# yichuan-w/LEANN

Hardware: AMD Instinct MI355X
Metric: queries/sec at recall@10>=0.9, 1M-chunk HNSW, MiniLM-L6 recompute (higher is better)
Workload: dtype fp16

## Files before the change

### include/leann_mi355x.h

```cpp
#ifndef LEANN_MI355X_H
#define LEANN_MI355X_H

#include <stddef.h>
#include <stdint.h>

#ifdef __cplusplus
extern "C" {
#endif

#define LM_OK 0
#define LM_EINVAL (-1)
#define LM_ENOENT (-2)
#define LM_EFORMAT (-3)
#define LM_EHIP (-4)
#define LM_ESTATE (-5)
#define LM_EPROVIDER (-6)

#define LM_METRIC_INNER_PRODUCT 0
#define LM_METRIC_L2 1

#define LM_DTYPE_F32 0
#define LM_DTYPE_F16 1

typedef struct lm_index lm_index;
typedef struct lm_tokens lm_tokens;

const char *lm_last_error(void);
int lm_device_count(void);
const char *lm_version(void);
#define LM_ABI_REVISION 6
int lm_abi_revision(void);

int lm_index_read(const char *path, int device, lm_index **out);

int lm_index_create_from_csr(int64_t ntotal, int32_t d, int32_t metric,
                             const uint64_t *node_offsets ,
                             const uint64_t *level_ptr, int64_t n_level_ptr,
                             const int32_t *neighbors, int64_t n_neighbors,
                             const int32_t *levels ,
                             int32_t entry_point, int32_t max_level, int device, lm_index **out);

typedef struct {
    const int32_t *d_nodes;
    const int32_t *d_adj;
    int64_t n_rows;
    int32_t cap;
} lm_graph_level;
int lm_index_create_view(int64_t ntotal, int32_t d, int32_t metric, const lm_graph_level *levels ,
                         int32_t n_levels, int32_t entry_point, int device, lm_index **out);
void lm_index_free(lm_index *idx);

typedef struct {
    int64_t ntotal;
    int32_t d;
    int32_t d_padded;
    int32_t metric;
    int32_t entry_point;
    int32_t max_level;
    int32_t max_degree0;
    int32_t max_degree_up;
    int64_t n_neighbors;
    int32_t has_table;
    int32_t has_provider;
    int32_t device;
} lm_index_info_t;
int lm_index_info(const lm_index *idx, lm_index_info_t *out);

int lm_index_attach_table(lm_index *idx, const void *table, int32_t dtype, int64_t ntotal, int32_t d,
                          int32_t location);

typedef int (*lm_provider_fn)(void *user, const int32_t *d_ids, int32_t n, void **d_out, void *stream);
int lm_index_set_provider(lm_index *idx, lm_provider_fn fn, void *user);

int lm_index_set_hub_cache(lm_index *idx, const int32_t *ids, int32_t n, const float *d_embeddings);

int lm_index_set_stream(lm_index *idx, void *hip_stream);

typedef struct {
    int32_t efSearch;
    int32_t beam_size;
    int32_t check_relative_distance;
    float pq_pruning_ratio;
    int32_t local_prune;
    float send_neigh_times_ratio;
    int32_t batch_size;
    int32_t zmq_port;
    int32_t recompute;
    int32_t max_batch;
    int32_t recompute_memo;
} lm_search_params;
void lm_search_params_default(lm_search_params *p);

int lm_index_search(lm_index *idx, int64_t n, const float *x, int32_t k, float *distances,
                    int64_t *labels, const lm_search_params *params);
int lm_index_search_device(lm_index *idx, int64_t n, const float *d_x, int32_t k, float *d_distances,
                           int64_t *d_labels, const lm_search_params *params);

typedef struct {
    int64_t ndis;
    int64_t nunique;
    int64_t nrounds;
    int64_t nexpand;
    int64_t update_launches;
    double update_ms;
    double expand_ms;
    double provider_ms;
    int64_t nadc;
    double update_span_ms;
    int64_t update_span_launches;
} lm_search_stats;
int lm_index_get_stats(const lm_index *idx, lm_search_stats *out);
int lm_index_set_profiling(lm_index *idx, int32_t enable);
int lm_index_event_overhead_us(lm_index *idx, double *out_us);
int lm_index_set_option(lm_index *idx, const char *name, int64_t value);
int lm_index_get_option(const lm_index *idx, const char *name, int64_t *value);

int lm_pq_attach(lm_index *idx, int32_t m, const float *codebooks, const uint8_t *codes, int64_t ntotal);
int lm_pq_attach_chunked(lm_index *idx, int32_t m, const int32_t *chunk_offsets, const float *codebooks, const uint8_t *codes,
                         int64_t ntotal);
typedef struct {
    int32_t complexity;
    int32_t beam_width;
    int32_t num_threads;
    int32_t use_deferred_fetch;
    int32_t skip_search_reorder;
    int32_t recompute_neighbors;
    int32_t dedup_node_dis;
    float prune_ratio;
    int32_t batch_recompute;
    int32_t use_global_pruning;
} lm_pq_search_params;
void lm_pq_search_params_default(lm_pq_search_params *p);
int lm_pq_batch_search(lm_index *idx, int64_t n, const float *x, int32_t k, const lm_pq_search_params *params,
                       int64_t *labels, float *distances);
int lm_pq_batch_search_device(lm_index *idx, int64_t n, const float *d_x, int32_t k,
                              const lm_pq_search_params *params, int64_t *d_labels, float *d_distances);

int lm_dist_gather(const void *d_table, int32_t dtype, int32_t d_padded, int32_t metric,
                   const float *d_q, const int32_t *d_qidx, const int32_t *d_ids, int64_t npairs,
                   float *d_out, void *stream);
int lm_topk_merge(const int64_t *d_in_ids, const float *d_in_dist, int32_t S, int32_t B, int32_t k,
                  int32_t metric, int64_t *d_out_ids, float *d_out_dist, void *stream);
#define LM_SELECT_MAX_K 512
int lm_select_neighbors(const void *d_table, int32_t dtype, int64_t ntable, int32_t d_padded, int32_t metric,
                        const int32_t *d_cand, const float *d_dist, int64_t n, int32_t K, int32_t m, float alpha,
                        uint8_t *d_keep, void *stream);
#define LM_LINK_STAGE 128
size_t lm_graph_add_links_workspace_bytes(int64_t n, int64_t ne);
int lm_graph_add_links(const void *d_table, int32_t dtype, int32_t d_padded, int32_t metric, int32_t *d_adj, float *d_dist,
                       int32_t *d_deg, int64_t n, int32_t cap, const int32_t *d_src, const int32_t *d_dst, const float *d_w, int64_t ne,
                       float alpha, void *d_workspace, size_t workspace_bytes, void *stream);
size_t lm_graph_prune_hubs_workspace_bytes(int64_t n, int32_t cap, int32_t m_low, int64_t n_hubs);
int lm_graph_prune_hubs(const void *d_table, int32_t dtype, int32_t d_padded, int32_t metric, const int32_t *d_adj_in, int64_t n,
                        int32_t cap, int32_t m_low, int64_t n_hubs, float alpha, int32_t *d_adj_out, float *d_dist_out,
                        int32_t *d_deg_out, int32_t *d_hubs , int32_t *d_indeg ,
                        void *d_workspace, size_t workspace_bytes, void *stream);
int lm_graph_insert_batch(lm_index *view, const int32_t *d_batch, int64_t b, int32_t replace, int32_t kk, int32_t m, float alpha,
                          const lm_search_params *params, int32_t *d_adj, float *d_dist, int32_t *d_deg,
                          int32_t *d_cand_out , float *d_cdist_out , uint8_t *d_keep_out );
#define LM_EXACT_MAX_K 256
size_t lm_exact_search_workspace_bytes(int64_t ntable, int64_t nq, int32_t k);
int lm_exact_search(const void *d_table, int32_t dtype, int64_t ntable, int32_t d_padded, int32_t metric, const float *d_q, int64_t nq,
                    int32_t k, const uint32_t *d_allow, float *d_distances, int64_t *d_labels, void *d_workspace, size_t workspace_bytes,
                    void *stream);
int lm_index_search_exact(lm_index *idx, int64_t n, const float *x, int32_t k, const uint32_t *allow, float *distances, int64_t *labels);
int lm_index_search_exact_device(lm_index *idx, int64_t n, const float *d_x, int32_t k, const uint32_t *d_allow, float *d_distances,
                                 int64_t *d_labels);
int lm_index_search_filtered(lm_index *idx, int64_t n, const float *x, int32_t k, const uint32_t *allow, float *distances, int64_t *labels,
                             const lm_search_params *params);
int lm_index_search_filtered_device(lm_index *idx, int64_t n, const float *d_x, int32_t k, const uint32_t *d_allow, float *d_distances,
                                    int64_t *d_labels, const lm_search_params *params);
#define LM_PQ_FLAT_MAX_L 1024
size_t lm_pq_scan_workspace_bytes(int64_t ntotal, int64_t nq, int32_t m, int32_t L);
int lm_pq_scan(const uint8_t *d_codes, int64_t ntotal, int32_t m, const int32_t *chunk_offsets, const float *d_codebooks, int32_t d,
               int32_t metric, const float *d_q, int64_t nq, int32_t ldq, int32_t L, const uint32_t *d_allow, float *d_distances,
               int64_t *d_labels, void *d_workspace, size_t workspace_bytes, void *stream);
int lm_pq_flat_search(lm_index *idx, int64_t n, const float *x, int32_t k, const lm_pq_search_params *params, const uint32_t *allow,
                      int64_t *labels, float *distances);
int lm_pq_flat_search_device(lm_index *idx, int64_t n, const float *d_x, int32_t k, const lm_pq_search_params *params,
                             const uint32_t *d_allow, int64_t *d_labels, float *d_distances);
int lm_pq_batch_search_filtered(lm_index *idx, int64_t n, const float *x, int32_t k, const lm_pq_search_params *params,
                                const uint32_t *allow, int64_t *labels, float *distances);
int lm_pq_batch_search_filtered_device(lm_index *idx, int64_t n, const float *d_x, int32_t k, const lm_pq_search_params *params,
                                       const uint32_t *d_allow, int64_t *d_labels, float *d_distances);
#define LM_PQ_MAX_SUB 64
int lm_pq_encode(const void *d_x, int32_t dtype, int64_t n, int32_t ld, int32_t d, int32_t m, const int32_t *chunk_offsets,
                 const float *d_codebooks, uint8_t *d_codes, void *stream);
int lm_pq_train(const void *d_x, int32_t dtype, int64_t s, int32_t ld, int32_t d, int32_t m, const int32_t *chunk_offsets,
                int32_t iters, float *d_codebooks, void *d_workspace, size_t workspace_bytes, void *stream);
size_t lm_pq_train_workspace_bytes(int64_t s, int32_t d, int32_t m);

int lm_add_layernorm_f16(const void *d_x, const void *d_residual, const void *d_gamma, const void *d_beta,
                         void *d_out, int64_t rows, int32_t hidden, float eps, void *stream);

int lm_attn_varlen_hd32_f16(const void *d_qkv, const int32_t *d_cu_seqlens, int32_t n_seqs, int32_t heads,
                            int32_t max_len, void *d_out, void *stream);

int lm_attn_varlen_f16(const void *d_qkv, const int32_t *d_cu_seqlens, int32_t n_seqs, int32_t heads, int32_t head_dim,
                       int32_t max_len, void *d_out, void *stream);

int lm_embed_layernorm_f16(const int32_t *d_tok, const int32_t *d_pos, const void *d_word, const void *d_pos_table,
                           const void *d_type0, const void *d_gamma, const void *d_beta, void *d_out, int64_t rows,
                           int32_t hidden, float eps, void *stream);

int lm_pack_tokens(const int32_t *d_ids, const int32_t *d_lens, const int32_t *d_cu_seqlens, int32_t n, int32_t t,
                   int32_t *d_tok, int32_t *d_pos, void *stream);

int lm_meanpool_varlen_f16(const void *d_x, const int32_t *d_cu_seqlens, int32_t n_seqs, int32_t hidden,
                           int32_t normalize, float *d_out, void *stream);

int lm_layer_tail_h384_f16(const void *d_attn, const void *d_resid, const void *d_wo_img, const float *d_bo,
                           const void *d_gamma1, const void *d_beta1, float eps1, const void *d_w1_img, const float *d_b1,
                           const void *d_w2_img, const float *d_b2, const void *d_gamma, const void *d_beta, void *d_out,
                           int64_t tokens, int32_t ffn, float eps, void *stream);
int lm_layer_tail_pack_h384(const void *d_wo_slabs, const void *d_w1_acc, const void *d_w2_slabs, int32_t ffn, void *d_wo_img,
                            void *d_w1_img, void *d_w2_img, void *stream);

int lm_qkv_attn_h384_f16(const void *d_x, const void *d_wqkv_img, const float *d_bqkv, const int32_t *d_cu_seqlens, int32_t n_seqs, int32_t max_len,
                         int64_t total_tokens, void *d_out, void *stream);
int lm_h384_first_half_form(int32_t heads, int32_t max_len, int64_t total_tokens, int32_t n_seqs);

int lm_qkv_h384_f16(const void *d_x, const void *d_w_img, const float *d_bias, int32_t n_out, void *d_out, int64_t tokens,
                    void *stream);
int lm_qkv_pack_h384(const void *d_w, int32_t n_out, void *d_w_img, void *stream);

int lm_gemm_ws_h384_f16(const void *d_x, const void *d_w, const float *d_bias, int32_t n_out, void *d_out, int64_t tokens,
                        void *stream);

int lm_gemm_f16(const void *d_x, const void *d_w, const float *d_bias, const void *d_residual, int32_t epilogue, int32_t n_out,
                int32_t k_in, void *d_out, int64_t tokens, void *stream);

typedef struct lm_bert_h384_layer {
    const void *wqkv;
    const float *bqkv;
    const void *wo_img;
    const float *bo;
    const void *ln1_gamma, *ln1_beta;
    const void *w1_img;
    const float *b1;
    const void *w2_img;
    const float *b2;
    const void *ln2_gamma, *ln2_beta;
    const void *wo, *w1, *w2;
    const void *wqkv_img;
} lm_bert_h384_layer;
#define LM_BERT_SMALL_TOKENS 8192
#define LM_BERT_QKV_GEMM_TOKENS 45056

typedef struct lm_bert_h384 {
    int32_t n_layers, heads, ffn, normalize;
    int32_t pooling;
    float ln_eps;
    const void *word, *pos_table, *type0, *emb_gamma, *emb_beta;
    const lm_bert_h384_layer *layers;
} lm_bert_h384;

size_t lm_bert_h384_workspace_bytes(int64_t total_tokens);
int lm_bert_h384_forward_packed(const lm_bert_h384 *m, const int32_t *d_tok, const int32_t *d_pos, const int32_t *d_cu_seqlens,
                                int32_t n_seqs, int64_t total_tokens, int32_t max_len, void *d_workspace, size_t workspace_bytes,
                                float *d_out, void *stream);

typedef struct lm_bert_layer {
    const void *wqkv;
    const float *bqkv;
    const void *wo;
    const float *bo;
    const void *ln1_gamma, *ln1_beta;
    const void *w1;
    const float *b1;
    const void *w2;
    const float *b2;
    const void *ln2_gamma, *ln2_beta;
} lm_bert_layer;

typedef struct lm_bert {
    int32_t hidden, n_layers, heads, ffn;
    int32_t pooling;
    int32_t normalize;
    float ln_eps;
    const void *word, *pos_table, *type0, *emb_gamma, *emb_beta;
    const lm_bert_layer *layers;
} lm_bert;

size_t lm_bert_workspace_bytes(const lm_bert *m, int64_t total_tokens);
int lm_bert_forward_packed(const lm_bert *m, const int32_t *d_tok, const int32_t *d_pos, const int32_t *d_cu_seqlens, int32_t n_seqs,
                           int64_t total_tokens, int32_t max_len, void *d_workspace, size_t workspace_bytes, float *d_out, void *stream);
int lm_clspool_varlen_f16(const void *d_x, const int32_t *d_cu_seqlens, int32_t n_seqs, int32_t hidden, int32_t normalize,
                          float *d_out, void *stream);

int lm_tokens_create(const uint16_t *tokens, const uint64_t *offsets , int64_t n, int device,
                     lm_tokens **out);
void lm_tokens_free(lm_tokens *t);
int lm_tokens_gather(const lm_tokens *t, const int32_t *d_ids, int32_t n, int32_t T, int32_t pad_id,
                     int32_t *d_out_ids, int32_t *d_out_len, void *stream);
int64_t lm_tokens_count(const lm_tokens *t);

typedef struct lm_recompute lm_recompute;
typedef struct lm_recompute_stats {
    int64_t calls, chunks, tokens, forwards, host_syncs;
} lm_recompute_stats;
int lm_recompute_create(const lm_bert_h384 *model, const lm_tokens *tokens, int32_t max_seq_len, int64_t max_tokens_per_forward,
                        lm_recompute **out);
int lm_recompute_create_general(const lm_bert *model, const lm_tokens *tokens, int32_t max_seq_len, int64_t max_tokens_per_forward,
                                lm_recompute **out);
void lm_recompute_free(lm_recompute *rc);
int lm_recompute_provider(void *user, const int32_t *d_ids, int32_t n, void **d_out, void *stream);
int lm_recompute_embed(lm_recompute *rc, const int32_t *d_ids, int32_t n, float *d_out, void *stream);
int lm_recompute_get_stats(const lm_recompute *rc, lm_recompute_stats *out);
int lm_index_set_recompute(lm_index *idx, lm_recompute *rc);

#define LM_KT_LAYER_TAIL 0
#define LM_KT_GEMM_WS 1
#define LM_KT_ATTN 2
#define LM_KT_GEMM_F16 3
#define LM_KT_QKV 4
#define LM_KT_QKV_ATTN 5
#define LM_KT_COUNT 6
typedef struct lm_kernel_time {
    const char *name;
    int64_t launches;
    double ms, work;
} lm_kernel_time;
int lm_kernel_timing_enable(uint32_t mask);
int lm_kernel_timing_read(lm_kernel_time *out, int32_t capacity, int32_t reset);

#ifdef __cplusplus
}
#endif
#endif
```

### leann_amd/_lib.py

```python

from __future__ import annotations

import ctypes as C
from pathlib import Path

_PKG = Path(__file__).resolve().parent
LIB_PATH = _PKG / "lib" / "libleann_mi355x.so"
BUILD_LIB_PATH = _PKG / "lib" / "libleann_hnswbuild.so"

LM_OK, LM_EINVAL, LM_ENOENT, LM_EFORMAT, LM_EHIP, LM_ESTATE, LM_EPROVIDER = 0, -1, -2, -3, -4, -5, -6
METRIC_INNER_PRODUCT, METRIC_L2 = 0, 1
DTYPE_F32, DTYPE_F16 = 0, 1
SELECT_MAX_K = 512
PQ_MAX_SUB = 64
EXACT_MAX_K = 256
LINK_STAGE = 128
PQ_FLAT_MAX_L = 1024


class LeannMi355xError(RuntimeError):
    pass


class IndexInfo(C.Structure):
    _fields_ = [
        ("ntotal", C.c_int64), ("d", C.c_int32), ("d_padded", C.c_int32), ("metric", C.c_int32),
        ("entry_point", C.c_int32), ("max_level", C.c_int32), ("max_degree0", C.c_int32),
        ("max_degree_up", C.c_int32), ("n_neighbors", C.c_int64), ("has_table", C.c_int32),
        ("has_provider", C.c_int32), ("device", C.c_int32),
    ]


class GraphLevel(C.Structure):
    _fields_ = [("d_nodes", C.c_void_p), ("d_adj", C.c_void_p), ("n_rows", C.c_int64), ("cap", C.c_int32)]


class SearchParams(C.Structure):

    _fields_ = [
        ("efSearch", C.c_int32), ("beam_size", C.c_int32), ("check_relative_distance", C.c_int32),
        ("pq_pruning_ratio", C.c_float), ("local_prune", C.c_int32), ("send_neigh_times_ratio", C.c_float),
        ("batch_size", C.c_int32), ("zmq_port", C.c_int32), ("recompute", C.c_int32), ("max_batch", C.c_int32),
        ("recompute_memo", C.c_int32),
    ]


class SearchStats(C.Structure):
    _fields_ = [
        ("ndis", C.c_int64), ("nunique", C.c_int64), ("nrounds", C.c_int64), ("nexpand", C.c_int64),
        ("update_launches", C.c_int64), ("update_ms", C.c_double), ("expand_ms", C.c_double),
        ("provider_ms", C.c_double), ("nadc", C.c_int64), ("update_span_ms", C.c_double), ("update_span_launches", C.c_int64),
    ]


class PqSearchParams(C.Structure):

    _fields_ = [
        ("complexity", C.c_int32), ("beam_width", C.c_int32), ("num_threads", C.c_int32),
        ("use_deferred_fetch", C.c_int32), ("skip_search_reorder", C.c_int32), ("recompute_neighbors", C.c_int32),
        ("dedup_node_dis", C.c_int32), ("prune_ratio", C.c_float), ("batch_recompute", C.c_int32),
        ("use_global_pruning", C.c_int32),
    ]


class BertH384Layer(C.Structure):
    _fields_ = [(n, C.c_void_p) for n in ("wqkv", "bqkv", "wo_img", "bo", "ln1_gamma", "ln1_beta", "w1_img", "b1", "w2_img", "b2", "ln2_gamma", "ln2_beta",
                                          "wo", "w1", "w2", "wqkv_img")]


class BertH384(C.Structure):
    _fields_ = [("n_layers", C.c_int32), ("heads", C.c_int32), ("ffn", C.c_int32), ("normalize", C.c_int32), ("pooling", C.c_int32), ("ln_eps", C.c_float),
                ("word", C.c_void_p), ("pos_table", C.c_void_p), ("type0", C.c_void_p), ("emb_gamma", C.c_void_p), ("emb_beta", C.c_void_p),
                ("layers", C.POINTER(BertH384Layer))]


class BertLayer(C.Structure):
    _fields_ = [(n, C.c_void_p) for n in ("wqkv", "bqkv", "wo", "bo", "ln1_gamma", "ln1_beta", "w1", "b1", "w2", "b2", "ln2_gamma", "ln2_beta")]


class Bert(C.Structure):
    _fields_ = [("hidden", C.c_int32), ("n_layers", C.c_int32), ("heads", C.c_int32), ("ffn", C.c_int32), ("pooling", C.c_int32),
                ("normalize", C.c_int32), ("ln_eps", C.c_float),
                ("word", C.c_void_p), ("pos_table", C.c_void_p), ("type0", C.c_void_p), ("emb_gamma", C.c_void_p), ("emb_beta", C.c_void_p),
                ("layers", C.POINTER(BertLayer))]


class KernelTime(C.Structure):
    _fields_ = [("name", C.c_char_p), ("launches", C.c_int64), ("ms", C.c_double), ("work", C.c_double)]


KT_LAYER_TAIL, KT_GEMM_WS, KT_ATTN, KT_GEMM_F16, KT_QKV, KT_QKV_ATTN, KT_COUNT = 0, 1, 2, 3, 4, 5, 6


class RecomputeStats(C.Structure):
    _fields_ = [(n, C.c_int64) for n in ("calls", "chunks", "tokens", "forwards", "host_syncs")]


ABI_REVISION = 6

PROVIDER_FN = C.CFUNCTYPE(C.c_int, C.c_void_p, C.c_void_p, C.c_int32, C.POINTER(C.c_void_p), C.c_void_p)

EXPORTED_SYMBOLS = [
    "lm_last_error", "lm_device_count", "lm_version", "lm_abi_revision",
    "lm_index_read", "lm_index_create_from_csr", "lm_index_create_view", "lm_index_free", "lm_index_info",
    "lm_index_attach_table", "lm_index_set_provider", "lm_index_set_hub_cache", "lm_index_set_stream",
    "lm_search_params_default", "lm_index_search", "lm_index_search_device",
    "lm_index_get_stats", "lm_index_set_profiling", "lm_index_set_option", "lm_index_get_option", "lm_index_event_overhead_us",
    "lm_dist_gather", "lm_topk_merge", "lm_select_neighbors", "lm_graph_add_links", "lm_graph_add_links_workspace_bytes", "lm_graph_prune_hubs", "lm_graph_prune_hubs_workspace_bytes", "lm_graph_insert_batch", "lm_pq_encode", "lm_pq_train", "lm_pq_train_workspace_bytes",
    "lm_exact_search", "lm_exact_search_workspace_bytes", "lm_index_search_exact", "lm_index_search_exact_device",
    "lm_index_search_filtered", "lm_index_search_filtered_device",
    "lm_pq_scan", "lm_pq_scan_workspace_bytes", "lm_pq_flat_search", "lm_pq_flat_search_device",
    "lm_pq_attach", "lm_pq_attach_chunked", "lm_pq_search_params_default", "lm_pq_batch_search", "lm_pq_batch_search_device",
    "lm_pq_batch_search_filtered", "lm_pq_batch_search_filtered_device",
    "lm_add_layernorm_f16", "lm_attn_varlen_hd32_f16", "lm_attn_varlen_f16", "lm_embed_layernorm_f16", "lm_meanpool_varlen_f16",
    "lm_layer_tail_h384_f16", "lm_layer_tail_pack_h384", "lm_qkv_h384_f16", "lm_qkv_attn_h384_f16", "lm_h384_first_half_form", "lm_qkv_pack_h384", "lm_gemm_ws_h384_f16", "lm_gemm_f16", "lm_pack_tokens",
    "lm_tokens_create", "lm_tokens_free", "lm_tokens_gather", "lm_tokens_count",
    "lm_bert_h384_workspace_bytes", "lm_bert_h384_forward_packed",
    "lm_bert_workspace_bytes", "lm_bert_forward_packed", "lm_clspool_varlen_f16",
    "lm_recompute_create", "lm_recompute_create_general", "lm_recompute_free", "lm_recompute_provider", "lm_recompute_embed", "lm_recompute_get_stats", "lm_index_set_recompute",
    "lm_kernel_timing_enable", "lm_kernel_timing_read",
]

_lib = None


def load() -> C.CDLL:
    global _lib
    if _lib is not None:
        return _lib
    if not LIB_PATH.exists():
        raise LeannMi355xError(
            f"{LIB_PATH} is missing: build it with `python -c 'import __graft_entry__ as g; g.build()'` "
            "or `make -C leann_amd/csrc`. leann-backend-mi355x has no CPU fallback."
        )
    lib = C.CDLL(str(LIB_PATH))
    vp, i32, i64, f32p = C.c_void_p, C.c_int32, C.c_int64, C.c_void_p
    lib.lm_last_error.restype = C.c_char_p
    lib.lm_version.restype = C.c_char_p
    if lib.lm_abi_revision() != ABI_REVISION:
        raise LeannMi355xError(f"{LIB_PATH} speaks ABI revision {lib.lm_abi_revision()}, this package was written against {ABI_REVISION}: rebuild it "
                               "(`make -C leann_amd/csrc`)")
    lib.lm_device_count.restype = C.c_int
    lib.lm_index_read.argtypes = [C.c_char_p, C.c_int, C.POINTER(vp)]
    lib.lm_index_create_from_csr.argtypes = [i64, i32, i32, vp, vp, i64, vp, i64, vp, i32, i32, C.c_int, C.POINTER(vp)]
    lib.lm_index_create_view.argtypes = [i64, i32, i32, C.POINTER(GraphLevel), i32, i32, C.c_int, C.POINTER(vp)]
    lib.lm_index_free.argtypes = [vp]
    lib.lm_index_free.restype = None
    lib.lm_index_info.argtypes = [vp, C.POINTER(IndexInfo)]
    lib.lm_index_attach_table.argtypes = [vp, vp, i32, i64, i32, i32]
    lib.lm_index_set_provider.argtypes = [vp, PROVIDER_FN, vp]
    lib.lm_index_set_stream.argtypes = [vp, vp]
    lib.lm_index_set_hub_cache.argtypes = [vp, vp, i32, vp]
    lib.lm_search_params_default.argtypes = [C.POINTER(SearchParams)]
    lib.lm_search_params_default.restype = None
    lib.lm_index_search.argtypes = [vp, i64, f32p, i32, vp, vp, C.POINTER(SearchParams)]
    lib.lm_index_search_device.argtypes = [vp, i64, vp, i32, vp, vp, C.POINTER(SearchParams)]
    lib.lm_index_get_stats.argtypes = [vp, C.POINTER(SearchStats)]
    lib.lm_index_set_profiling.argtypes = [vp, i32]
    lib.lm_index_set_option.argtypes = [vp, C.c_char_p, i64]
    lib.lm_index_get_option.argtypes = [vp, C.c_char_p, C.POINTER(C.c_int64)]
    lib.lm_index_event_overhead_us.argtypes = [vp, C.POINTER(C.c_double)]
    lib.lm_dist_gather.argtypes = [vp, i32, i32, i32, vp, vp, vp, i64, vp, vp]
    lib.lm_topk_merge.argtypes = [vp, vp, i32, i32, i32, i32, vp, vp, vp]
    lib.lm_select_neighbors.argtypes = [vp, i32, i64, i32, i32, vp, vp, i64, i32, i32, C.c_float, vp, vp]
    lib.lm_graph_add_links_workspace_bytes.argtypes = [i64, i64]
    lib.lm_graph_add_links_workspace_bytes.restype = C.c_size_t
    lib.lm_graph_add_links.argtypes = [vp, i32, i32, i32, vp, vp, vp, i64, i32, vp, vp, vp, i64, C.c_float, vp, C.c_size_t, vp]
    lib.lm_graph_prune_hubs_workspace_bytes.argtypes = [i64, i32, i32, i64]
    lib.lm_graph_prune_hubs_workspace_bytes.restype = C.c_size_t
    lib.lm_graph_prune_hubs.argtypes = [vp, i32, i32, i32, vp, i64, i32, i32, i64, C.c_float, vp, vp, vp, vp, vp, vp, C.c_size_t, vp]
    lib.lm_graph_insert_batch.argtypes = [vp, vp, i64, i32, i32, i32, C.c_float, C.POINTER(SearchParams), vp, vp, vp, vp, vp, vp]
    lib.lm_pq_encode.argtypes = [vp, i32, i64, i32, i32, i32, vp, vp, vp, vp]
    lib.lm_pq_train.argtypes = [vp, i32, i64, i32, i32, i32, vp, i32, vp, vp, C.c_size_t, vp]
    lib.lm_pq_train_workspace_bytes.argtypes = [i64, i32, i32]
    lib.lm_pq_train_workspace_bytes.restype = C.c_size_t
    lib.lm_exact_search_workspace_bytes.argtypes = [i64, i64, i32]
    lib.lm_exact_search_workspace_bytes.restype = C.c_size_t
    lib.lm_exact_search.argtypes = [vp, i32, i64, i32, i32, vp, i64, i32, vp, vp, vp, vp, C.c_size_t, vp]
    lib.lm_index_search_exact.argtypes = [vp, i64, vp, i32, vp, vp, vp]
    lib.lm_index_search_exact_device.argtypes = [vp, i64, vp, i32, vp, vp, vp]
    lib.lm_index_search_filtered.argtypes = [vp, i64, vp, i32, vp, vp, vp, C.POINTER(SearchParams)]
    lib.lm_index_search_filtered_device.argtypes = [vp, i64, vp, i32, vp, vp, vp, C.POINTER(SearchParams)]
    lib.lm_pq_scan_workspace_bytes.argtypes = [i64, i64, i32, i32]
    lib.lm_pq_scan_workspace_bytes.restype = C.c_size_t
    lib.lm_pq_scan.argtypes = [vp, i64, i32, vp, vp, i32, i32, vp, i64, i32, i32, vp, vp, vp, vp, C.c_size_t, vp]
    lib.lm_pq_flat_search.argtypes = [vp, i64, vp, i32, C.POINTER(PqSearchParams), vp, vp, vp]
    lib.lm_pq_flat_search_device.argtypes = [vp, i64, vp, i32, C.POINTER(PqSearchParams), vp, vp, vp]
    lib.lm_pq_attach.argtypes = [vp, i32, vp, vp, i64]
    lib.lm_pq_attach_chunked.argtypes = [vp, i32, vp, vp, vp, i64]
    lib.lm_pq_search_params_default.argtypes = [C.POINTER(PqSearchParams)]
    lib.lm_pq_search_params_default.restype = None
    lib.lm_pq_batch_search.argtypes = [vp, i64, vp, i32, C.POINTER(PqSearchParams), vp, vp]
    lib.lm_pq_batch_search_device.argtypes = [vp, i64, vp, i32, C.POINTER(PqSearchParams), vp, vp]
    lib.lm_pq_batch_search_filtered.argtypes = [vp, i64, vp, i32, C.POINTER(PqSearchParams), vp, vp, vp]
    lib.lm_pq_batch_search_filtered_device.argtypes = [vp, i64, vp, i32, C.POINTER(PqSearchParams), vp, vp, vp]
    lib.lm_add_layernorm_f16.argtypes = [vp, vp, vp, vp, vp, i64, i32, C.c_float, vp]
    lib.lm_attn_varlen_hd32_f16.argtypes = [vp, vp, i32, i32, i32, vp, vp]
    lib.lm_attn_varlen_f16.argtypes = [vp, vp, i32, i32, i32, i32, vp, vp]
    lib.lm_embed_layernorm_f16.argtypes = [vp, vp, vp, vp, vp, vp, vp, vp, i64, i32, C.c_float, vp]
    lib.lm_meanpool_varlen_f16.argtypes = [vp, vp, i32, i32, i32, vp, vp]
    lib.lm_layer_tail_h384_f16.argtypes = [vp, vp, vp, vp, vp, vp, C.c_float, vp, vp, vp, vp, vp, vp, vp, i64, i32, C.c_float, vp]
    lib.lm_layer_tail_pack_h384.argtypes = [vp, vp, vp, i32, vp, vp, vp, vp]
    lib.lm_qkv_h384_f16.argtypes = [vp, vp, vp, i32, vp, i64, vp]
    lib.lm_qkv_attn_h384_f16.argtypes = [vp, vp, vp, vp, i32, i32, i64, vp, vp]
    lib.lm_h384_first_half_form.argtypes = [i32, i32, i64, i32]
    lib.lm_qkv_pack_h384.argtypes = [vp, i32, vp, vp]
    lib.lm_gemm_ws_h384_f16.argtypes = [vp, vp, vp, i32, vp, i64, vp]
    lib.lm_gemm_f16.argtypes = [vp, vp, vp, vp, i32, i32, i32, vp, i64, vp]
    lib.lm_pack_tokens.argtypes = [vp, vp, vp, i32, i32, vp, vp, vp]
    lib.lm_tokens_create.argtypes = [vp, vp, i64, C.c_int, C.POINTER(vp)]
    lib.lm_tokens_free.argtypes = [vp]
    lib.lm_tokens_free.restype = None
    lib.lm_tokens_gather.argtypes = [vp, vp, i32, i32, i32, vp, vp, vp]
    lib.lm_tokens_count.argtypes = [vp]
    lib.lm_tokens_count.restype = i64
    lib.lm_bert_h384_workspace_bytes.argtypes = [i64]
    lib.lm_bert_h384_workspace_bytes.restype = C.c_size_t
    lib.lm_bert_h384_forward_packed.argtypes = [C.POINTER(BertH384), vp, vp, vp, i32, i64, i32, vp, C.c_size_t, vp, vp]
    lib.lm_bert_workspace_bytes.argtypes = [C.POINTER(Bert), i64]
    lib.lm_bert_workspace_bytes.restype = C.c_size_t
    lib.lm_bert_forward_packed.argtypes = [C.POINTER(Bert), vp, vp, vp, i32, i64, i32, vp, C.c_size_t, vp, vp]
    lib.lm_clspool_varlen_f16.argtypes = [vp, vp, i32, i32, i32, vp, vp]
    lib.lm_recompute_create.argtypes = [C.POINTER(BertH384), vp, i32, i64, C.POINTER(vp)]
    lib.lm_recompute_create_general.argtypes = [C.POINTER(Bert), vp, i32, i64, C.POINTER(vp)]
    lib.lm_recompute_free.argtypes = [vp]
    lib.lm_recompute_free.restype = None
    lib.lm_recompute_provider.argtypes = [vp, vp, i32, C.POINTER(vp), vp]
    lib.lm_recompute_embed.argtypes = [vp, vp, i32, vp, vp]
    lib.lm_recompute_get_stats.argtypes = [vp, C.POINTER(RecomputeStats)]
    lib.lm_index_set_recompute.argtypes = [vp, vp]
    lib.lm_kernel_timing_enable.argtypes = [C.c_uint32]
    lib.lm_kernel_timing_read.argtypes = [C.POINTER(KernelTime), i32, i32]
    _lib = lib
    return lib


def last_error() -> str:
    return (load().lm_last_error() or b"").decode("utf-8", "replace")


def check(rc: int, what: str = "") -> None:
    if rc == LM_OK:
        return
    msg = f"{what}: {last_error()}" if what else last_error()
    if rc == LM_EINVAL or rc == LM_EFORMAT:
        raise ValueError(msg)
    if rc == LM_ENOENT:
        raise FileNotFoundError(msg)
    raise LeannMi355xError(msg)


def kernel_timing_enable(mask: int) -> None:
    check(load().lm_kernel_timing_enable(int(mask)), "lm_kernel_timing_enable")


def kernel_timing_read(reset: bool = False) -> dict:
    arr = (KernelTime * KT_COUNT)()
    check(load().lm_kernel_timing_read(arr, KT_COUNT, 1 if reset else 0), "lm_kernel_timing_read")
    return {a.name.decode(): {"launches": int(a.launches), "ms": float(a.ms), "work": float(a.work)} for a in arr}


def device_count() -> int:
    return int(load().lm_device_count())


def require_gpu() -> None:
    if device_count() <= 0:
        raise LeannMi355xError("no HIP device visible: leann-backend-mi355x needs an MI355X (gfx950) GPU and has no CPU fallback")
```

### leann_amd/csrc/lm_device_types.h

```cpp
#pragma once

namespace lm {

struct L0Range {
    uint64_t begin;
    uint32_t count;
    uint32_t pad;
};

struct GraphDev {
    int64_t N;
    int32_t entry_point, max_level;
    const uint64_t* node_offsets;
    const uint64_t* level_ptr;
    const int32_t* neighbors;
    const L0Range* l0;
};

struct WsDev {
    int32_t B, ef, W, maxnew;
    int32_t efs;
    int32_t batch;
    int32_t check_rel;
    int64_t nw;
    int32_t* phase;
    int32_t* level;
    uint64_t* cur_key;
    int32_t* nsteps;
    int32_t* npool;
    int32_t* npop;
    int32_t* nnew;
    unsigned long long* ndis_q;
    int32_t* pop;
    int32_t* newid;
    uint64_t* pool;
    uint32_t* visited;
    uint32_t* rbm;
    uint32_t* rbm_snap;
    int32_t* word_rank;
    int32_t* tile_sum;
    int32_t* uniq;
    uint64_t* aq;
    int32_t* naq;
    unsigned long long* nadc_q;
    int32_t* memo_slot;
    float* memo;
    unsigned long long* counters;
};
enum { C_LIVE = 0, C_NUNIQ = 1, C_NDIS = 2, C_NEXPAND = 3, C_ROUNDS = 4, C_RC_TOKENS = 5, C_NADC = 6, C_RC_MAXLEN = 7, C_PQ_OVERFLOW = 8, C_PQ_ALLOWED = 9, C_NCOUNTERS = 10 };

constexpr int UNIQ_TILE = 4096;
constexpr int AQ_CAP = 512;


}
```

### leann_amd/csrc/lm_encoder_forward.cpp

```cpp
#include <algorithm>
#include <cstdint>
#include <cstdlib>
#include <string>

#include "lm_internal.h"

static int64_t small_tokens_limit() {
    const char* e = getenv("LEANN_MI355X_SMALL_TOKENS");
    return e ? (int64_t)atoll(e) : (int64_t)LM_BERT_SMALL_TOKENS;
}

lm::H384FirstHalf lm::h384_first_half_form(int32_t heads, int32_t max_len, int64_t total_tokens, int32_t n_seqs) {
    auto is = [](const char* name, char c) {
        const char* e = getenv(name);
        return e && e[0] == c;
    };
    if (heads != 12 || max_len > 256) return H384_PAIR_ROW_MAJOR;
    if (is("LEANN_MI355X_QKV_LAYOUT", '0') || is("LEANN_MI355X_ATTN3", '9') || is("LEANN_MI355X_ATTN", '2')) return H384_PAIR_ROW_MAJOR;
    if (is("LEANN_MI355X_FUSED_QKV_ATTN", '0')) return H384_PAIR_HEAD_MAJOR;
    if (is("LEANN_MI355X_FUSED_QKV_ATTN", '1')) return H384_FUSED;
    return n_seqs > 0 && total_tokens >= (int64_t)H384_FUSED_MIN_MEAN_LEN * n_seqs ? H384_FUSED : H384_PAIR_HEAD_MAJOR;
}
extern "C" int lm_h384_first_half_form(int32_t heads, int32_t max_len, int64_t total_tokens, int32_t n_seqs) {
    return (int)lm::h384_first_half_form(heads, max_len, total_tokens, n_seqs);
}

static int64_t qkv_gemm_tokens_limit() {
    if (const char* e = getenv("LEANN_MI355X_QKV_GEMM_TOKENS")) return (int64_t)atoll(e);
    const char* s = getenv("LEANN_MI355X_SMALL_TOKENS");
    return s && atoll(s) == 0 ? 0 : (int64_t)LM_BERT_QKV_GEMM_TOKENS;
}

extern "C" size_t lm_bert_h384_workspace_bytes(int64_t total_tokens) {
    if (total_tokens <= 0) return 0;
    const size_t small = total_tokens <= std::max<int64_t>(small_tokens_limit(), LM_BERT_SMALL_TOKENS) ? (size_t)total_tokens * 2560 * 2 : 0;
    return (size_t)total_tokens * (3 * 384 + 1152) * 2 + small;
}

extern "C" int lm_bert_h384_forward_packed(const lm_bert_h384* m, const int32_t* d_tok, const int32_t* d_pos, const int32_t* d_cu_seqlens,
                                           int32_t n_seqs, int64_t total_tokens, int32_t max_len, void* d_workspace, size_t workspace_bytes,
                                           float* d_out, void* stream) {
    using namespace lm;
    if (n_seqs == 0 || total_tokens == 0) return LM_OK;
    if (!m || !m->layers || !d_tok || !d_pos || !d_cu_seqlens || !d_workspace || !d_out || n_seqs < 0 || total_tokens < 0)
        LM_FAIL(LM_EINVAL, "lm_bert_h384_forward_packed: bad arguments");
    if (!bert_h384_envelope_ok(m->n_layers, m->heads, m->ffn)) LM_FAIL(LM_EINVAL, "lm_bert_h384_forward_packed: needs " LM_BERT_H384_ENVELOPE_TEXT);
    if (max_len <= 0 || max_len > 256) LM_FAIL(LM_EINVAL, "lm_bert_h384_forward_packed: sequence lengths 1..256");
    if (m->pooling != 0 && m->pooling != 1) LM_FAIL(LM_EINVAL, "lm_bert_h384_forward_packed: pooling 0 (mean) or 1 (CLS)");
    if (workspace_bytes < lm_bert_h384_workspace_bytes(total_tokens)) LM_FAIL(LM_EINVAL, "lm_bert_h384_forward_packed: workspace too small");
    const size_t row = (size_t)total_tokens * 384 * 2;
    unsigned char* ws = (unsigned char*)d_workspace;
    void* x = ws;
    void* a = ws + row;
    void* y = ws + 2 * row;
    void* qkv = ws + 3 * row;
    int rc = lm_embed_layernorm_f16(d_tok, d_pos, m->word, m->pos_table, m->type0, m->emb_gamma, m->emb_beta, x, total_tokens, 384, m->ln_eps, stream);
    if (rc) return rc;
    bool small = total_tokens <= small_tokens_limit() && m->ffn % 128 == 0;
    for (int l = 0; small && l < m->n_layers; ++l) small = m->layers[l].wo && m->layers[l].w1 && m->layers[l].w2;
    void* hid = ws + 3 * row + (size_t)total_tokens * 1152 * 2;
    H384FirstHalf first_half = h384_first_half_form(m->heads, max_len, total_tokens, n_seqs);
    bool qkv_gemm = !small && total_tokens <= qkv_gemm_tokens_limit();
    for (int l = 0; qkv_gemm && l < m->n_layers; ++l) qkv_gemm = m->layers[l].wqkv != nullptr;
    {
        const char* f = getenv("LEANN_MI355X_FUSED_QKV_ATTN");
        if (qkv_gemm && f && f[0] == '1') qkv_gemm = false;
        else if (qkv_gemm) first_half = H384_PAIR_ROW_MAJOR;
    }
    for (int l = 0; l < m->n_layers; ++l) {
        const lm_bert_h384_layer& L = m->layers[l];
        if (small) {
            if ((rc = lm_gemm_f16(x, L.wqkv, L.bqkv, nullptr, 0, 1152, 384, qkv, total_tokens, stream))) return rc;
            if ((rc = lm_attn_varlen_hd32_f16(qkv, d_cu_seqlens, n_seqs, m->heads, max_len, a, stream))) return rc;
            if ((rc = lm_gemm_f16(a, L.wo, L.bo, x, 2, 384, 384, y, total_tokens, stream))) return rc;
            if ((rc = lm_add_layernorm_f16(y, nullptr, L.ln1_gamma, L.ln1_beta, x, total_tokens, 384, m->ln_eps, stream))) return rc;
            if ((rc = lm_gemm_f16(x, L.w1, L.b1, nullptr, 1, m->ffn, 384, hid, total_tokens, stream))) return rc;
            if ((rc = lm_gemm_f16(hid, L.w2, L.b2, x, 2, 384, m->ffn, y, total_tokens, stream))) return rc;
            if ((rc = lm_add_layernorm_f16(y, nullptr, L.ln2_gamma, L.ln2_beta, x, total_tokens, 384, m->ln_eps, stream))) return rc;
            continue;
        }
        if (L.wqkv_img && first_half == H384_FUSED) {
            if ((rc = lm_qkv_attn_h384_launch(x, L.wqkv_img, L.bqkv, d_cu_seqlens, n_seqs, max_len, total_tokens, a, stream))) return rc;
        } else if (L.wqkv_img && first_half == H384_PAIR_HEAD_MAJOR) {
            if ((rc = lm_qkv_h384_launch(x, L.wqkv_img, L.bqkv, 1152, qkv, total_tokens, 1, stream))) return rc;
            if ((rc = lm_attn_v3_launch_hd32(qkv, d_cu_seqlens, n_seqs, m->heads, max_len, a, total_tokens, stream))) return rc;
        } else {
            if ((rc = qkv_gemm      ? lm_gemm_f16(x, L.wqkv, L.bqkv, nullptr, 0, 1152, 384, qkv, total_tokens, stream)
                      : L.wqkv_img ? lm_qkv_h384_f16(x, L.wqkv_img, L.bqkv, 1152, qkv, total_tokens, stream)
                                   : lm_gemm_ws_h384_f16(x, L.wqkv, L.bqkv, 1152, qkv, total_tokens, stream)))
                return rc;
            if ((rc = lm_attn_varlen_hd32_f16(qkv, d_cu_seqlens, n_seqs, m->heads, max_len, a, stream))) return rc;
        }
        if ((rc = lm_layer_tail_h384_f16(a, x, L.wo_img, L.bo, L.ln1_gamma, L.ln1_beta, m->ln_eps, L.w1_img, L.b1, L.w2_img, L.b2, L.ln2_gamma,
                                         L.ln2_beta, y, total_tokens, m->ffn, m->ln_eps, stream)))
            return rc;
        void* t = x;
        x = y;
        y = t;
    }
    return m->pooling == 1 ? lm_clspool_varlen_f16(x, d_cu_seqlens, n_seqs, 384, m->normalize, d_out, stream)
                           : lm_meanpool_varlen_f16(x, d_cu_seqlens, n_seqs, 384, m->normalize, d_out, stream);
}

static const char* bert_envelope(const lm_bert* m) {
    if (!m || !m->layers || m->n_layers <= 0) return "NULL model / no layers";
    if (m->hidden <= 0 || m->hidden % 128 || m->hidden > 768) return "hidden must be a multiple of 128, <= 768";
    if (m->ffn <= 0 || m->ffn % 128) return "ffn must be a multiple of 128";
    if (m->heads <= 0 || (m->heads * 32 != m->hidden && m->heads * 64 != m->hidden)) return "head_dim = hidden / heads must be 32 or 64";
    if (m->pooling != 0 && m->pooling != 1) return "pooling: 0 = mean, 1 = CLS";
    return nullptr;
}

extern "C" size_t lm_bert_workspace_bytes(const lm_bert* m, int64_t total_tokens) {
    if (!m || total_tokens <= 0) return 0;
    return (size_t)total_tokens * ((size_t)6 * m->hidden + m->ffn) * 2;
}

extern "C" int lm_bert_forward_packed(const lm_bert* m, const int32_t* d_tok, const int32_t* d_pos, const int32_t* d_cu_seqlens, int32_t n_seqs,
                                      int64_t total_tokens, int32_t max_len, void* d_workspace, size_t workspace_bytes, float* d_out,
                                      void* stream) {
    using namespace lm;
    if (n_seqs == 0 || total_tokens == 0) return LM_OK;
    if (const char* why = bert_envelope(m)) LM_FAIL(LM_EINVAL, std::string("lm_bert_forward_packed: ") + why);
    if (!d_tok || !d_pos || !d_cu_seqlens || !d_workspace || !d_out || n_seqs < 0 || total_tokens < 0)
        LM_FAIL(LM_EINVAL, "lm_bert_forward_packed: bad arguments");
    const int32_t H = m->hidden, hd = H / m->heads;
    if (max_len <= 0 || max_len > (hd == 32 ? 256 : 512)) LM_FAIL(LM_EINVAL, "lm_bert_forward_packed: sequence lengths 1..256 (head_dim 32) / 1..512 (head_dim 64)");
    if (workspace_bytes < lm_bert_workspace_bytes(m, total_tokens)) LM_FAIL(LM_EINVAL, "lm_bert_forward_packed: workspace too small");
    const size_t row = (size_t)total_tokens * H * 2;
    unsigned char* ws = (unsigned char*)d_workspace;
    void *x = ws, *a = ws + row, *y = ws + 2 * row, *qkv = ws + 3 * row, *hid = ws + 6 * row;
    int rc = lm_embed_layernorm_f16(d_tok, d_pos, m->word, m->pos_table, m->type0, m->emb_gamma, m->emb_beta, x, total_tokens, H, m->ln_eps, stream);
    if (rc) return rc;
    for (int l = 0; l < m->n_layers; ++l) {
        const lm_bert_layer& L = m->layers[l];
        if ((rc = lm_gemm_f16(x, L.wqkv, L.bqkv, nullptr, 0, 3 * H, H, qkv, total_tokens, stream))) return rc;
        if ((rc = hd == 32 ? lm_attn_varlen_hd32_f16(qkv, d_cu_seqlens, n_seqs, m->heads, max_len, a, stream)
                           : lm_attn_varlen_f16(qkv, d_cu_seqlens, n_seqs, m->heads, hd, max_len, a, stream)))
            return rc;
        if ((rc = lm_gemm_f16(a, L.wo, L.bo, x, 2, H, H, y, total_tokens, stream))) return rc;
        if ((rc = lm_add_layernorm_f16(y, nullptr, L.ln1_gamma, L.ln1_beta, x, total_tokens, H, m->ln_eps, stream))) return rc;
        if ((rc = lm_gemm_f16(x, L.w1, L.b1, nullptr, 1, m->ffn, H, hid, total_tokens, stream))) return rc;
        if ((rc = lm_gemm_f16(hid, L.w2, L.b2, x, 2, H, m->ffn, y, total_tokens, stream))) return rc;
        if ((rc = lm_add_layernorm_f16(y, nullptr, L.ln2_gamma, L.ln2_beta, x, total_tokens, H, m->ln_eps, stream))) return rc;
    }
    return m->pooling == 1 ? lm_clspool_varlen_f16(x, d_cu_seqlens, n_seqs, H, m->normalize, d_out, stream)
                           : lm_meanpool_varlen_f16(x, d_cu_seqlens, n_seqs, H, m->normalize, d_out, stream);
}
```

### leann_amd/csrc/lm_internal.h

```cpp
#pragma once
#include <hip/hip_runtime.h>

#include <cstdint>
#include <cstdio>
#include <string>
#include <vector>

#include "../../include/leann_mi355x.h"

namespace lm {

void set_error(const std::string& msg);

#define LM_HIP(expr)                                                                       \
    do {                                                                                   \
        hipError_t _e = (expr);                                                            \
        if (_e != hipSuccess) {                                                            \
            lm::set_error(std::string(#expr) + ": " + hipGetErrorString(_e));              \
            return LM_EHIP;                                                                \
        }                                                                                  \
    } while (0)

#ifndef LM_KEEP_LOCAL
#define LM_KEEP_LOCAL(v) asm volatile("" : "+v"(v))
#endif

#ifndef LM_ONE_WAVE_PER_SIMD
#define LM_ONE_WAVE_PER_SIMD __attribute__((amdgpu_waves_per_eu(1, 1)))
#endif
#ifndef LM_TWO_WAVES_PER_SIMD
#define LM_TWO_WAVES_PER_SIMD __attribute__((amdgpu_waves_per_eu(2, 2)))
#endif

#ifndef LM_WAVE_SYNC
#define LM_WAVE_SYNC() ((void)0)
#endif

#define LM_FAIL(code, msg)        \
    do {                          \
        lm::set_error(msg);       \
        return (code);            \
    } while (0)

struct DynLdsAttr {
    size_t bytes[32] = {};
};
inline hipError_t ensure_dyn_lds(DynLdsAttr& a, const void* fn, size_t bytes) {
    int dev = 0;
    if (hipGetDevice(&dev) != hipSuccess || dev < 0) dev = 0;
    size_t& have = a.bytes[dev & 31];
    if (bytes <= have && dev < 32) return hipSuccess;
    hipError_t e = hipFuncSetAttribute(fn, hipFuncAttributeMaxDynamicSharedMemorySize, (int)bytes);
    if (e == hipSuccess) have = bytes;
    return e;
}

struct KtScope {
    int kid;
    void* st;
    double work;
    void* a;
    int dev;
    KtScope(int kid, void* stream, double work);
    ~KtScope();
    KtScope(const KtScope&) = delete;
    KtScope& operator=(const KtScope&) = delete;
};

void kt_attn_work(const int32_t* d_cu_seqlens, int32_t n_seqs, int32_t hidden, void* stream, int kid = LM_KT_ATTN);

enum : int32_t { PH_SEED = 0, PH_UPPER = 1, PH_BEAM = 2, PH_DONE = 3 };

constexpr uint64_t KEY_NONE = 0xFFFFFFFFFFFFFFFFull;
constexpr uint64_t KEY_EXPANDED = 1ull;

__host__ __device__ inline uint64_t make_key(float d, int32_t id) {
    if (d != d) d = __builtin_inff();
    if (d == 0.0f) d = 0.0f;
    uint32_t u = __builtin_bit_cast(uint32_t, d);
    u ^= (u >> 31) ? 0xFFFFFFFFu : 0x80000000u;
    return ((uint64_t)u << 32) | ((uint64_t)(uint32_t)id << 1);
}
__host__ __device__ inline float key_dist(uint64_t key) {
    uint32_t u = (uint32_t)(key >> 32);
    u ^= (u >> 31) ? 0x80000000u : 0xFFFFFFFFu;
    return __builtin_bit_cast(float, u);
}
__host__ __device__ inline int32_t key_id(uint64_t key) { return (int32_t)((uint32_t)key >> 1); }

struct HostCsr {
    int64_t ntotal = 0;
    int32_t d = 0;
    int32_t metric = 0;
    int32_t entry_point = -1;
    int32_t max_level = -1;
    std::vector<int32_t> levels;
    std::vector<uint64_t> level_ptr;
    std::vector<uint64_t> node_offsets;
    std::vector<int32_t> neighbors;
    std::vector<float> storage;
};
int read_csr_file(const char* path, HostCsr& out);

}

struct lm_tokens {
    int device = 0;
    int64_t n = 0;
    uint64_t total = 0;
    uint16_t* d_tok = nullptr;
    uint64_t* d_off = nullptr;
};

struct lm_recompute;
namespace lm {
int rc_prepare(lm_recompute* rc, const int32_t* d_ids, const unsigned long long* d_n, int64_t cap, unsigned long long* d_total,
               unsigned long long* d_maxlen, hipStream_t st);
void rc_prepared(lm_recompute* rc, const int32_t* d_ids, int32_t n, int64_t total, int32_t max_len);
int32_t rc_width(const lm_recompute* rc);
inline bool bert_h384_envelope_ok(int n_layers, int heads, int ffn) { return n_layers > 0 && heads * 32 == 384 && ffn >= 192 && ffn <= 1728 && ffn % 192 == 0; }
#define LM_BERT_H384_ENVELOPE_TEXT "hidden 384 = heads x 32 and ffn a multiple of 192 in [192, 1728]"
enum H384FirstHalf : int { H384_FUSED = 0, H384_PAIR_HEAD_MAJOR = 1, H384_PAIR_ROW_MAJOR = 2 };
constexpr int H384_FUSED_MIN_MEAN_LEN = 216;
H384FirstHalf h384_first_half_form(int32_t heads, int32_t max_len, int64_t total_tokens, int32_t n_seqs);

}

int lm_qkv_h384_launch(const void* d_x, const void* d_w_img, const float* d_bias, int32_t n_out, void* d_out, int64_t tokens, int32_t head_major, void* stream);

int lm_attn_v3_launch_hd32(const void* d_qkv, const int32_t* d_cu_seqlens, int32_t n_seqs, int32_t heads, int32_t max_len, void* d_out, int64_t total_tokens,
                           void* stream);

int lm_qkv_attn_h384_launch(const void* d_x, const void* d_wqkv_img, const float* d_bqkv, const int32_t* d_cu_seqlens, int32_t n_seqs, int32_t max_len,
                            int64_t total_tokens, void* d_out, void* stream);

int lm_add_layernorm_r16_launch(const void* d_x, const void* d_residual, const void* d_gamma, const void* d_beta, void* d_out,
                                int64_t rows, int32_t hidden, float eps, void* stream);
```

### leann_amd/csrc/lm_recompute.hip

```cpp
#include <algorithm>
#include <climits>
#include <cstdlib>
#include <cstring>

#include "lm_device_types.h"
#include "lm_internal.h"

struct lm_recompute {
    int device = 0;
    lm_bert_h384 model{};
    std::vector<lm_bert_h384_layer> layers;
    bool general = false;
    lm_bert gmodel{};
    std::vector<lm_bert_layer> glayers;
    int32_t hidden = 384;
    const lm_tokens* tokens = nullptr;
    int32_t T = 0;
    int64_t max_tokens = 0;
    int32_t* d_cu = nullptr;
    int32_t* d_cu_sub = nullptr;
    int64_t cu_cap = 0;
    int32_t* d_tok = nullptr;
    int64_t tok_cap = 0;
    void* d_ws = nullptr;
    size_t ws_bytes = 0;
    float* d_out = nullptr;
    int64_t out_cap = 0;
    unsigned long long* d_meta = nullptr;
    unsigned long long* h_meta = nullptr;
    std::vector<int32_t> h_cu;
    const int32_t* prep_ids = nullptr;
    int32_t prep_n = -1;
    int64_t prep_total = 0;
    int32_t prep_maxlen = 0;
    bool prep_launched = false;
    int64_t chunks = 0, tokens_seen = 0, forwards = 0, calls = 0, syncs = 0;
};

namespace lm {

__global__ __launch_bounds__(1024) void k_rc_lengths_scan(const uint64_t* __restrict__ off, const int32_t* __restrict__ ids, int32_t n_host,
                                                          const unsigned long long* __restrict__ d_n, int64_t cap, int32_t T,
                                                          int32_t* __restrict__ cu, unsigned long long* __restrict__ out_total,
                                                          unsigned long long* __restrict__ out_maxlen) {
    __shared__ int32_t s_wave[16];
    __shared__ int32_t s_max[16];
    const int tid = threadIdx.x, lane = tid & 63, wave = tid >> 6;
    int64_t n = d_n ? (int64_t)*d_n : (int64_t)n_host;
    if (n > cap) n = cap;
    int32_t carry = 0, mx = 0;
    auto length_of = [&](int64_t i) -> int32_t {
        if (i >= n) return 0;
        const int32_t id = ids[i];
        const uint64_t b = off[id], e = off[id + 1];
        return (int32_t)min((uint64_t)T, e - b);
    };
    int32_t len = length_of(tid);
    for (int64_t base = 0; base < n; base += 1024) {
        const int32_t nxt = length_of(base + 1024 + tid);
        int32_t v = len;
        mx = max(mx, len);
        for (int d = 1; d < 64; d <<= 1) {
            const int32_t t = __shfl_up(v, d);
            if (lane >= d) v += t;
        }
        if (lane == 63) s_wave[wave] = v;
        __syncthreads();
        int32_t before = 0, block_total = 0;
#pragma unroll
        for (int w = 0; w < 16; ++w) {
            const int32_t s = s_wave[w];
            before += w < wave ? s : 0;
            block_total += s;
        }
        if (base + tid < n) cu[base + tid + 1] = carry + before + v;
        carry += block_total;
        len = nxt;
        __syncthreads();
    }
    for (int d = 32; d >= 1; d >>= 1) mx = max(mx, __shfl_xor(mx, d));
    if (lane == 0) s_max[wave] = mx;
    __syncthreads();
    if (tid == 0) {
        int32_t m = 0;
        for (int w = 0; w < 16; ++w) m = max(m, s_max[w]);
        cu[0] = 0;
        *out_total = (unsigned long long)(uint32_t)carry;
        *out_maxlen = (unsigned long long)(uint32_t)m;
    }
}

__global__ __launch_bounds__(256) void k_rc_pack(const uint16_t* __restrict__ tok, const uint64_t* __restrict__ off,
                                                 const int32_t* __restrict__ ids, const int32_t* __restrict__ cu, int32_t b0, int32_t n_sub,
                                                 int32_t* __restrict__ out_tok, int32_t* __restrict__ out_pos, int32_t* __restrict__ cu_sub) {
    const int w = blockIdx.x * 4 + (threadIdx.x >> 6), lane = threadIdx.x & 63;
    if (w >= n_sub) return;
    const int32_t first = cu[b0], lo = cu[b0 + w], hi = cu[b0 + w + 1];
    const int32_t base = lo - first, len = hi - lo;
    const uint64_t src = off[ids[b0 + w]];
    for (int j = lane; j < len; j += 64) {
        out_tok[base + j] = (int32_t)tok[src + j];
        out_pos[base + j] = j;
    }
    if (lane == 0) {
        cu_sub[w] = base;
        if (w == n_sub - 1) cu_sub[n_sub] = hi - first;
    }
}

template <typename P>
static int rc_grow(lm_recompute* rc, P** p, int64_t* cap, int64_t need, size_t elem, hipStream_t st, int64_t at_least = 1024) {
    if (need <= *cap) return LM_OK;
    if (*p) {
        LM_HIP(hipStreamSynchronize(st));
        rc->syncs++;
        (void)hipFree(*p);
        *p = nullptr;
        *cap = 0;
    }
    const int64_t want = (std::max<int64_t>(need + need / 4, at_least) + 1) & ~(int64_t)1;
    void* v = nullptr;
    LM_HIP(hipMalloc(&v, (size_t)want * elem));
    *p = (P*)v;
    *cap = want;
    return LM_OK;
}

static int rc_ensure_cu(lm_recompute* rc, int64_t n, hipStream_t st) {
    int r = rc_grow(rc, &rc->d_cu, &rc->cu_cap, 2 * (n + 1), 4, st);
    rc->d_cu_sub = rc->d_cu + rc->cu_cap / 2;
    return r;
}

int rc_prepare(lm_recompute* rc, const int32_t* d_ids, const unsigned long long* d_n, int64_t cap, unsigned long long* d_total,
               unsigned long long* d_maxlen, hipStream_t st) {
    rc->prep_ids = nullptr;
    rc->prep_n = -1;
    rc->prep_launched = false;
    if (cap * (int64_t)rc->T > (int64_t)INT32_MAX) return LM_OK;
    int r = rc_ensure_cu(rc, cap, st);
    if (r) return r;
    hipLaunchKernelGGL(k_rc_lengths_scan, dim3(1), dim3(1024), 0, st, rc->tokens->d_off, d_ids, 0, d_n, cap, rc->T, rc->d_cu, d_total, d_maxlen);
    LM_HIP(hipGetLastError());
    rc->prep_launched = true;
    return LM_OK;
}

void rc_prepared(lm_recompute* rc, const int32_t* d_ids, int32_t n, int64_t total, int32_t max_len) {
    if (!rc->prep_launched) return;
    rc->prep_launched = false;
    rc->prep_ids = d_ids;
    rc->prep_n = n;
    rc->prep_total = total;
    rc->prep_maxlen = max_len;
}

static int rc_forward(lm_recompute* rc, const int32_t* d_ids, int32_t b0, int32_t n_sub, int64_t total, int32_t max_len, float* d_out,
                      hipStream_t st) {
    int r;
    if ((r = rc_grow(rc, &rc->d_tok, &rc->tok_cap, 2 * total, 4, st, (int64_t)1 << 18))) return r;
    int32_t* d_pos = rc->d_tok + rc->tok_cap / 2;
    const size_t need = rc->general ? lm_bert_workspace_bytes(&rc->gmodel, total) : lm_bert_h384_workspace_bytes(total);
    if (need > rc->ws_bytes) {
        if (rc->d_ws) {
            LM_HIP(hipStreamSynchronize(st));
            rc->syncs++;
            (void)hipFree(rc->d_ws);
            rc->d_ws = nullptr;
            rc->ws_bytes = 0;
        }
        const size_t want = std::max<size_t>(need + need / 4, (size_t)64 << 20);
        LM_HIP(hipMalloc(&rc->d_ws, want));
        rc->ws_bytes = want;
    }
    hipLaunchKernelGGL(k_rc_pack, dim3((unsigned)((n_sub + 3) / 4)), dim3(256), 0, st, rc->tokens->d_tok, rc->tokens->d_off, d_ids, rc->d_cu, b0,
                       n_sub, rc->d_tok, d_pos, rc->d_cu_sub);
    LM_HIP(hipGetLastError());
    rc->forwards++;
    if (rc->general)
        return lm_bert_forward_packed(&rc->gmodel, rc->d_tok, d_pos, rc->d_cu_sub, n_sub, total, max_len, rc->d_ws, rc->ws_bytes, d_out, (void*)st);
    return lm_bert_h384_forward_packed(&rc->model, rc->d_tok, d_pos, rc->d_cu_sub, n_sub, total, max_len, rc->d_ws, rc->ws_bytes, d_out,
                                       (void*)st);
}

static int rc_embed(lm_recompute* rc, const int32_t* d_ids, int32_t n, float* d_out, hipStream_t st) {
    int r;
    rc->calls++;
    if (n == 0) return LM_OK;
    int64_t total;
    int32_t max_len;
    if (rc->prep_ids == d_ids && rc->prep_n == n) {
        total = rc->prep_total;
        max_len = rc->prep_maxlen;
    } else {
        if ((int64_t)n * rc->T > (int64_t)INT32_MAX) LM_FAIL(LM_EINVAL, "recompute provider: more than 2^31 tokens in one call");
        if ((r = rc_ensure_cu(rc, n, st))) return r;
        hipLaunchKernelGGL(k_rc_lengths_scan, dim3(1), dim3(1024), 0, st, rc->tokens->d_off, d_ids, n, (const unsigned long long*)nullptr,
                           (int64_t)n, rc->T, rc->d_cu, rc->d_meta, rc->d_meta + 1);
        LM_HIP(hipGetLastError());
        LM_HIP(hipMemcpyAsync(rc->h_meta, rc->d_meta, 16, hipMemcpyDeviceToHost, st));
        LM_HIP(hipStreamSynchronize(st));
        rc->syncs++;
        total = (int64_t)rc->h_meta[0];
        max_len = (int32_t)rc->h_meta[1];
    }
    rc->prep_ids = nullptr;
    rc->prep_n = -1;
    rc->chunks += n;
    rc->tokens_seen += total;
    if (total == 0) {
        LM_HIP(hipMemsetAsync(d_out, 0, (size_t)n * rc->hidden * 4, st));
        return LM_OK;
    }
    if (total <= rc->max_tokens) return rc_forward(rc, d_ids, 0, n, total, max_len, d_out, st);
    rc->h_cu.resize((size_t)n + 1);
    LM_HIP(hipMemcpyAsync(rc->h_cu.data(), rc->d_cu, ((size_t)n + 1) * 4, hipMemcpyDeviceToHost, st));
    LM_HIP(hipStreamSynchronize(st));
    rc->syncs++;
    const int32_t* cs = rc->h_cu.data();
    int32_t b0 = 0;
    while (b0 < n) {
        const int64_t limit = (int64_t)cs[b0] + rc->max_tokens;
        int32_t j = (int32_t)(std::upper_bound(cs + 1, cs + n + 1, limit, [](int64_t lim, int32_t v) { return lim < (int64_t)v; }) - (cs + 1));
        j = std::min(std::max(j, b0 + 1), n);
        int32_t ml = 0;
        for (int32_t i = b0; i < j; ++i) ml = std::max(ml, cs[i + 1] - cs[i]);
        const int64_t sub_total = (int64_t)cs[j] - cs[b0];
        if (sub_total > 0) {
            if ((r = rc_forward(rc, d_ids, b0, j - b0, sub_total, ml, d_out + (size_t)b0 * rc->hidden, st))) return r;
        } else {
            LM_HIP(hipMemsetAsync(d_out + (size_t)b0 * rc->hidden, 0, (size_t)(j - b0) * rc->hidden * 4, st));
        }
        b0 = j;
    }
    return LM_OK;
}

int32_t rc_width(const lm_recompute* rc) { return rc->hidden; }

static int rc_finish_create(lm_recompute* rc, const lm_tokens* tokens, int32_t max_seq_len, int64_t max_tokens, lm_recompute** out) {
    rc->device = tokens->device;
    rc->tokens = tokens;
    rc->T = max_seq_len;
    rc->max_tokens = max_tokens;
    if (const char* ft = getenv("LEANN_MI355X_FORWARD_TOKENS"))
        if (atoll(ft) > 0) rc->max_tokens = atoll(ft);
    hipError_t e;
    if ((e = hipMalloc((void**)&rc->d_meta, 16)) != hipSuccess || (e = hipHostMalloc((void**)&rc->h_meta, 16)) != hipSuccess) {
        set_error(std::string("lm_recompute_create: ") + hipGetErrorString(e));
        lm_recompute_free(rc);
        return LM_EHIP;
    }
    *out = rc;
    return LM_OK;
}

}

extern "C" {

int lm_recompute_create(const lm_bert_h384* model, const lm_tokens* tokens, int32_t max_seq_len, int64_t max_tokens_per_forward,
                        lm_recompute** out) {
    using namespace lm;
    if (!out) LM_FAIL(LM_EINVAL, "out is NULL");
    *out = nullptr;
    if (!model || !model->layers || !tokens) LM_FAIL(LM_EINVAL, "lm_recompute_create: NULL model / token store");
    if (!bert_h384_envelope_ok(model->n_layers, model->heads, model->ffn))
        LM_FAIL(LM_EINVAL, "lm_recompute_create: needs " LM_BERT_H384_ENVELOPE_TEXT " (the one-call forward's envelope; other shapes: lm_recompute_create_general)");
    if (max_seq_len <= 0 || max_seq_len > 256) LM_FAIL(LM_EINVAL, "lm_recompute_create: chunk length limit must be 1..256 tokens");
    if (max_tokens_per_forward <= 0) LM_FAIL(LM_EINVAL, "lm_recompute_create: max_tokens_per_forward must be positive");
    LM_HIP(hipSetDevice(tokens->device));
    lm_recompute* rc = new lm_recompute();
    rc->model = *model;
    rc->layers.assign(model->layers, model->layers + model->n_layers);
    rc->model.layers = rc->layers.data();
    return rc_finish_create(rc, tokens, max_seq_len, max_tokens_per_forward, out);
}

int lm_recompute_create_general(const lm_bert* model, const lm_tokens* tokens, int32_t max_seq_len, int64_t max_tokens_per_forward,
                                lm_recompute** out) {
    using namespace lm;
    if (!out) LM_FAIL(LM_EINVAL, "out is NULL");
    *out = nullptr;
    if (!model || !model->layers || !tokens) LM_FAIL(LM_EINVAL, "lm_recompute_create_general: NULL model / token store");
    if (model->n_layers <= 0 || model->hidden <= 0 || model->hidden % 128 || model->hidden > 768 || model->ffn <= 0 || model->ffn % 128 ||
        model->heads <= 0 || (model->heads * 32 != model->hidden && model->heads * 64 != model->hidden) || (model->pooling != 0 && model->pooling != 1))
        LM_FAIL(LM_EINVAL, "lm_recompute_create_general: outside lm_bert_forward_packed's envelope (hidden % 128 == 0 and <= 768, ffn % 128 == 0, "
                           "head_dim 32 or 64, mean or CLS pooling)");
    if (max_seq_len <= 0 || max_seq_len > (model->heads * 32 == model->hidden ? 256 : 512))
        LM_FAIL(LM_EINVAL, "lm_recompute_create_general: chunk length limit must be 1..256 tokens (head_dim 32) / 1..512 (head_dim 64)");
    if (max_tokens_per_forward <= 0) LM_FAIL(LM_EINVAL, "lm_recompute_create_general: max_tokens_per_forward must be positive");
    LM_HIP(hipSetDevice(tokens->device));
    lm_recompute* rc = new lm_recompute();
    rc->general = true;
    rc->gmodel = *model;
    rc->glayers.assign(model->layers, model->layers + model->n_layers);
    rc->gmodel.layers = rc->glayers.data();
    rc->hidden = model->hidden;
    return rc_finish_create(rc, tokens, max_seq_len, max_tokens_per_forward, out);
}

void lm_recompute_free(lm_recompute* rc) {
    if (!rc) return;
    (void)hipSetDevice(rc->device);
    for (void* p : {(void*)rc->d_cu, (void*)rc->d_tok, rc->d_ws, (void*)rc->d_out, (void*)rc->d_meta})
        if (p) (void)hipFree(p);
    if (rc->h_meta) (void)hipHostFree(rc->h_meta);
    delete rc;
}

int lm_recompute_provider(void* user, const int32_t* d_ids, int32_t n, void** d_out, void* stream) {
    using namespace lm;
    lm_recompute* rc = (lm_recompute*)user;
    if (!rc || !d_out || n < 0 || (n > 0 && !d_ids)) LM_FAIL(LM_EINVAL, "lm_recompute_provider: bad arguments");
    LM_HIP(hipSetDevice(rc->device));
    hipStream_t st = (hipStream_t)stream;
    int r = rc_grow(rc, &rc->d_out, &rc->out_cap, (int64_t)std::max(n, 1) * rc->hidden, 4, st, (int64_t)4096 * rc->hidden);
    if (r) return r;
    *d_out = rc->d_out;
    return rc_embed(rc, d_ids, n, rc->d_out, st);
}

int lm_recompute_embed(lm_recompute* rc, const int32_t* d_ids, int32_t n, float* d_out, void* stream) {
    using namespace lm;
    if (!rc || n < 0 || (n > 0 && (!d_ids || !d_out))) LM_FAIL(LM_EINVAL, "lm_recompute_embed: bad arguments");
    LM_HIP(hipSetDevice(rc->device));
    return rc_embed(rc, d_ids, n, d_out, (hipStream_t)stream);
}

int lm_recompute_get_stats(const lm_recompute* rc, lm_recompute_stats* out) {
    using namespace lm;
    if (!rc || !out) LM_FAIL(LM_EINVAL, "lm_recompute_get_stats: NULL argument");
    out->calls = rc->calls;
    out->chunks = rc->chunks;
    out->tokens = rc->tokens_seen;
    out->forwards = rc->forwards;
    out->host_syncs = rc->syncs;
    return LM_OK;
}

}
```

### leann_amd/csrc/lm_search.hip

```cpp
#include <algorithm>
#include <cmath>
#include <cstring>
#include <type_traits>

#include <hip/hip_fp16.h>

#include "lm_internal.h"
#include "lm_devbuf.h"

namespace lm {

static thread_local std::string g_err;
void set_error(const std::string& msg) { g_err = msg; }


}

#include "lm_device_types.h"
#include "lm_beam_common.h"
#include "lm_kernels_expand.h"
#include "lm_kernels_prune.h"
#include "lm_kernels_update.h"
#include "lm_view_impl.h"
#include "lm_kernels_persist.h"
#include "lm_kernels_misc.h"
#include "lm_filter_impl.h"


using namespace lm;

struct lm_index {
    int device = 0;
    int64_t N = 0;
    int32_t D = 0, Dp = 0, metric = 0, entry_point = -1, max_level = -1;
    int32_t maxdeg0 = 0, maxdeg_up = 0;
    int64_t n_neighbors = 0, n_level_ptr = 0;
    DevBuf<uint64_t> d_node_offsets, d_level_ptr;
    DevBuf<int32_t> d_neighbors;
    DevBuf<L0Range> d_l0;
    bool view = false;
    std::vector<lm_graph_level> view_levels;
    DevBuf<ViewLevelDev> d_view_up;
    int32_t pq_m = 0;
    DevBuf<float> d_pq_codebooks;
    DevBuf<uint8_t> d_pq_codes;
    DevBuf<int32_t> d_pq_chunk_off;
    DevBuf<float> d_stage_x, d_stage_d;
    DevBuf<int64_t> d_stage_l;
    DevBuf<uint32_t> d_allow;
    DevBuf<unsigned long long> d_pq_nadc;
    DevBuf<int32_t> d_pq_rounds;
    DevBuf<float> d_lut;
    DevBuf<unsigned long long> d_tstamp;
    double span_ms = 0;
    int64_t span_launches = 0;
    void* d_table = nullptr;
    bool table_owned = false;
    int32_t table_dtype = LM_DTYPE_F32;
    lm_provider_fn provider = nullptr;
    void* provider_user = nullptr;
    lm_recompute* native_rc = nullptr;
    hipStream_t stream = nullptr;
    WsDev ws{};
    int32_t ws_B = 0, ws_ef = 0, ws_W = 0, ws_maxnew = 0, ws_spec = 0;
    int64_t ws_ucap = 0;
    int single_query_direct = 0;
    int speculate = 0;
    int speculate_max_batch = 2;
    DevBuf<int32_t> d_memo_slot;
    float* d_memo = nullptr;
    int64_t memo_cap = 0;
    int64_t memo_initial_rows = 0;
    DevBuf<int32_t> d_hub_slot_init;
    int64_t hub_n = 0;
    std::vector<void*> ws_allocs;
    DevBuf<float> d_qpad;
    DevBuf<unsigned char> d_exact_ws, d_pqflat_ws, d_filter_ws;
    DevBuf<float> d_ins_q, d_ins_sd, d_ins_cdist, d_ins_w;
    DevBuf<int64_t> d_ins_sl;
    DevBuf<int32_t> d_ins_cand, d_ins_src, d_ins_dst;
    DevBuf<uint8_t> d_ins_keep;
    DevBuf<unsigned char> d_ins_ws;
    int64_t filtered_allowed_evals = 0;
    std::vector<int32_t> h_pq_chunk_off;
    unsigned long long* h_counters = nullptr;
    lm_search_stats stats{};
    bool profiling = false;
    int update_variant = 0;
    int persistent_table = 1;
    int pq_threads = 1024;
    bool pq_rerank_expanded = false;
    int64_t pq_overflow = 0;
    int persistent_wave = -1;
    int wave_maxnew = 0;
    double avg_degree0 = 0;
    std::vector<std::pair<hipEvent_t, hipEvent_t>> ev_update, ev_expand, ev_provider;
    std::vector<hipEvent_t> ev_pool;
};

#define LM_NOT_ON_VIEW(ix, what) \
    do { \
        if ((ix) && (ix)->view) LM_FAIL(LM_ESTATE, std::string(what) + " is not served by a view index (lm_index_create_view): build a CSR index for it"); \
    } while (0)

static int free_ws(lm_index* ix) {
    for (void* p : ix->ws_allocs) (void)hipFree(p);
    ix->ws_allocs.clear();
    ix->ws_B = ix->ws_ef = ix->ws_W = ix->ws_maxnew = ix->ws_spec = 0;
    ix->ws_ucap = 0;
    return 0;
}

template <typename T>
static int ws_alloc(lm_index* ix, T** p, size_t count) {
    void* v = nullptr;
    LM_HIP(hipMalloc(&v, std::max<size_t>(count, 1) * sizeof(T)));
    ix->ws_allocs.push_back(v);
    *p = (T*)v;
    return LM_OK;
}

static int64_t ws_maxnew(const lm_index* ix, int64_t W, bool prune, int64_t batch) {
    int64_t maxnew = std::max<int64_t>({W * ix->maxdeg0, (int64_t)ix->maxdeg_up, (int64_t)1});
    if (batch > 0) maxnew = std::max(maxnew, batch - 1 + ix->maxdeg0);
    if (prune) maxnew = std::max(maxnew, (int64_t)AQ_CAP);
    return maxnew;
}

static int64_t next_pow2_64(int64_t x) {
    int64_t p = 1;
    while (p < x) p <<= 1;
    return p;
}

static int ensure_ws(lm_index* ix, int32_t B, int32_t ef, int32_t W, bool prune = false, int32_t spec = 0, int32_t batch = 0) {
    const int64_t maxnew64 = ws_maxnew(ix, W, prune, batch);
    if (maxnew64 > (1 << 24)) LM_FAIL(LM_EINVAL, "beam_size / batch_size too large: a round's new-list would not fit the LDS");
    const int32_t maxnew = (int32_t)maxnew64;
    if (B <= ix->ws_B && ef == ix->ws_ef && W == ix->ws_W && maxnew == ix->ws_maxnew && spec == ix->ws_spec) {
        ix->ws.B = B;
        return LM_OK;
    }
    free_ws(ix);
    WsDev& w = ix->ws;
    w.B = B; w.ef = ef; w.W = W; w.maxnew = maxnew;
    w.nw = (ix->N + 31) / 32;
    int rc;
#define A(ptr, cnt) if ((rc = ws_alloc(ix, &w.ptr, (cnt))) != LM_OK) return rc
    A(phase, B); A(level, B); A(cur_key, B); A(nsteps, B); A(npool, B); A(npop, B); A(nnew, B); A(ndis_q, B);
    A(naq, B); A(nadc_q, B); A(aq, (size_t)B * AQ_CAP);
    A(pop, (size_t)B * W); A(newid, (size_t)B * maxnew); A(pool, (size_t)B * ef);
    A(visited, (size_t)B * w.nw);
    A(rbm, w.nw); A(rbm_snap, w.nw); A(word_rank, w.nw);
    int ntiles = (int)((w.nw + UNIQ_TILE - 1) / UNIQ_TILE);
    A(tile_sum, std::max(ntiles, 1));
    ix->ws_ucap = std::min<int64_t>(ix->N, (int64_t)B * (std::max(maxnew, ef) + (int64_t)spec * ix->maxdeg0));
    A(uniq, ix->ws_ucap);
    A(counters, C_NCOUNTERS);
#undef A
    LM_HIP(hipMemsetAsync(w.rbm, 0, w.nw * 4, ix->stream));
    ix->ws_B = B; ix->ws_ef = ef; ix->ws_W = W; ix->ws_maxnew = maxnew; ix->ws_spec = spec;
    return LM_OK;
}

static int ensure_memo_rows(lm_index* ix, int64_t need, int64_t keep) {
    if (need <= ix->memo_cap) return LM_OK;
    if (need > ix->N) LM_FAIL(LM_ESTATE, "internal: the embedding memo cannot need more rows than the index has nodes");
    const int64_t cap = std::min<int64_t>(ix->N, std::max<int64_t>({need, 2 * ix->memo_cap, (int64_t)65536}));
    float* grown = nullptr;
    if (hipMalloc((void**)&grown, (size_t)cap * ix->Dp * 4) != hipSuccess) {
        (void)hipGetLastError();
        LM_FAIL(LM_EHIP, "out of device memory for the per-call recompute memo (" + std::to_string((size_t)cap * ix->Dp * 4 >> 20) +
                             " MiB); search with recompute_memo = 0 or a smaller max_batch");
    }
    if (ix->d_memo) {
        if (keep > 0) LM_HIP(hipMemcpyAsync(grown, ix->d_memo, (size_t)keep * ix->Dp * 4, hipMemcpyDeviceToDevice, ix->stream));
        LM_HIP(hipStreamSynchronize(ix->stream));
        (void)hipFree(ix->d_memo);
    }
    ix->d_memo = grown;
    ix->memo_cap = cap;
    ix->ws.memo = grown;
    return LM_OK;
}

static int ensure_pq_counters(lm_index* ix, int32_t B) {
    if (int rc = ix->d_pq_nadc.reserve((size_t)B)) return rc;
    return ix->d_pq_rounds.reserve((size_t)B);
}

static int pad_queries(lm_index* ix, int64_t n, const float* d_x, const float** d_q) {
    *d_q = d_x;
    if (ix->D == ix->Dp) return LM_OK;
    const int64_t tot = n * ix->Dp;
    if (int rc = ix->d_qpad.reserve((size_t)tot)) return rc;
    hipLaunchKernelGGL(k_pad_rows, dim3((unsigned)((tot + 255) / 256)), dim3(256), 0, ix->stream, d_x, n, ix->D, ix->Dp, ix->d_qpad.get());
    *d_q = ix->d_qpad.get();
    return LM_OK;
}


static int upload_allow(lm_index* ix, const uint32_t* allow, const uint32_t** d_allow) {
    *d_allow = nullptr;
    if (!allow) return LM_OK;
    const size_t words = (size_t)((ix->N + 31) / 32);
    if (int rc = ix->d_allow.reserve(words, 4)) return rc;
    if (words) LM_HIP(hipMemcpyAsync(ix->d_allow.get(), allow, words * 4, hipMemcpyHostToDevice, ix->stream));
    *d_allow = ix->d_allow.get();
    return LM_OK;
}

static int stage_in(lm_index* ix, const float* x, int64_t n, int32_t k) {
    if (int rc = ix->d_stage_x.reserve((size_t)n * ix->D, 1024)) return rc;
    if (int rc = ix->d_stage_d.reserve((size_t)n * k, 1024)) return rc;
    if (int rc = ix->d_stage_l.reserve((size_t)n * k, 512)) return rc;
    LM_HIP(hipMemcpyAsync(ix->d_stage_x.get(), x, (size_t)n * ix->D * 4, hipMemcpyHostToDevice, ix->stream));
    return LM_OK;
}

static int stage_out(lm_index* ix, float* distances, int64_t* labels, int64_t n, int32_t k) {
    LM_HIP(hipMemcpyAsync(distances, ix->d_stage_d.get(), (size_t)n * k * 4, hipMemcpyDeviceToHost, ix->stream));
    LM_HIP(hipMemcpyAsync(labels, ix->d_stage_l.get(), (size_t)n * k * 8, hipMemcpyDeviceToHost, ix->stream));
    LM_HIP(hipStreamSynchronize(ix->stream));
    return LM_OK;
}

static hipEvent_t get_event(lm_index* ix) {
    hipEvent_t e;
    if (!ix->ev_pool.empty()) {
        e = ix->ev_pool.back();
        ix->ev_pool.pop_back();
        return e;
    }
    (void)hipEventCreate(&e);
    return e;
}

static double drain_events(lm_index* ix, std::vector<std::pair<hipEvent_t, hipEvent_t>>& v) {
    double ms = 0;
    for (auto& p : v) {
        float t = 0;
        if (hipEventElapsedTime(&t, p.first, p.second) == hipSuccess) ms += t;
        ix->ev_pool.push_back(p.first);
        ix->ev_pool.push_back(p.second);
    }
    v.clear();
    return ms;
}

struct EvScope {
    lm_index* ix;
    std::vector<std::pair<hipEvent_t, hipEvent_t>>* v;
    hipEvent_t a{}, b{};
    EvScope(lm_index* i, std::vector<std::pair<hipEvent_t, hipEvent_t>>* vec) : ix(i), v(vec) {
        if (ix->profiling) {
            a = get_event(ix);
            b = get_event(ix);
            (void)hipEventRecord(a, ix->stream);
        }
    }
    ~EvScope() {
        if (ix->profiling) {
            (void)hipEventRecord(b, ix->stream);
            v->push_back({a, b});
        }
    }
};

static int next_pow2(int x) {
    int p = 1;
    while (p < x) p <<= 1;
    return p;
}

template <bool L2, bool F16>
static int launch_update_nch(lm_index* ix, const UpdateArgs& a, size_t shmem) {
    dim3 grid(ix->ws.B), block(256);
    const bool wave = ix->update_variant == 3 ||
                      (ix->update_variant == 0 && ix->ws.B >= 4096 && ix->ws.W * ix->avg_degree0 <= (double)ix->wave_maxnew);
    switch (ix->Dp / 64) {
#define CASE(n)                                                                                              \
    case n:                                                                                                  \
        if (a.by_rank == 2) hipLaunchKernelGGL((k_update<n, L2, F16, 2, 256>), grid, block, shmem, ix->stream, ix->ws, a); \
        else if (wave && a.by_rank) hipLaunchKernelGGL((k_update<n, L2, F16, 1, 64>), grid, dim3(64), shmem, ix->stream, ix->ws, a); \
        else if (wave) hipLaunchKernelGGL((k_update<n, L2, F16, 0, 64>), grid, dim3(64), shmem, ix->stream, ix->ws, a); \
        else if (a.by_rank) hipLaunchKernelGGL((k_update<n, L2, F16, 1, 256>), grid, block, shmem, ix->stream, ix->ws, a); \
        else hipLaunchKernelGGL((k_update<n, L2, F16, 0, 256>), grid, block, shmem, ix->stream, ix->ws, a);   \
        break
        CASE(1); CASE(2); CASE(3); CASE(4); CASE(5); CASE(6); CASE(8); CASE(12); CASE(16);
#undef CASE
        default: LM_FAIL(LM_EINVAL, "unsupported padded dimension (supported: 64..384, 512, 768, 1024)");
    }
    LM_HIP(hipGetLastError());
    return LM_OK;
}

static int launch_update(lm_index* ix, const UpdateArgs& a, bool f16) {
    size_t shmem = (size_t)(2 * ix->ws.ef + next_pow2(ix->ws.maxnew)) * sizeof(uint64_t);
    bool l2 = ix->metric == LM_METRIC_L2;
    if (l2) return f16 ? launch_update_nch<true, true>(ix, a, shmem) : launch_update_nch<true, false>(ix, a, shmem);
    return f16 ? launch_update_nch<false, true>(ix, a, shmem) : launch_update_nch<false, false>(ix, a, shmem);
}

struct FilterPass {
    const uint32_t* d_allow;
    bool rounds_max = false;
};

static int ensure_filter_ws(lm_index* ix, int32_t B, int32_t k, FilterDev& f) {
    const size_t res_bytes = (size_t)B * k * 8, cnt_bytes = ((size_t)B + 1) * 8, len_bytes = (size_t)B * 4;
    if (int rc = ix->d_filter_ws.reserve(res_bytes + cnt_bytes + len_bytes)) return rc;
    unsigned char* p = ix->d_filter_ws.get();
    f.res = (uint64_t*)p;
    f.nallow = (unsigned long long*)(p + res_bytes);
    f.nres = (int32_t*)(p + res_bytes + cnt_bytes);
    f.k = k;
    return LM_OK;
}

static int launch_filter_collect(lm_index* ix, const UpdateArgs& a, bool f16, const FilterDev& f) {
    const size_t shmem = (size_t)(2 * f.k + next_pow2(ix->ws.maxnew)) * sizeof(uint64_t);
    const dim3 grid(ix->ws.B), block(256);
    const bool l2 = ix->metric == LM_METRIC_L2;
    switch (ix->Dp / 64) {
#define CASEF(n)                                                                                                            \
    case n:                                                                                                                 \
        if (l2 && f16) hipLaunchKernelGGL((k_filter_collect<n, true, true>), grid, block, shmem, ix->stream, ix->ws, a, f);   \
        else if (l2) hipLaunchKernelGGL((k_filter_collect<n, true, false>), grid, block, shmem, ix->stream, ix->ws, a, f);    \
        else if (f16) hipLaunchKernelGGL((k_filter_collect<n, false, true>), grid, block, shmem, ix->stream, ix->ws, a, f);   \
        else hipLaunchKernelGGL((k_filter_collect<n, false, false>), grid, block, shmem, ix->stream, ix->ws, a, f);           \
        break
        CASEF(1); CASEF(2); CASEF(3); CASEF(4); CASEF(5); CASEF(6); CASEF(8); CASEF(12); CASEF(16);
#undef CASEF
        default: LM_FAIL(LM_EINVAL, "unsupported padded dimension (supported: 64..384, 512, 768, 1024)");
    }
    LM_HIP(hipGetLastError());
    return LM_OK;
}

static bool persist_wave_form(const lm_index* ix) {
    if (ix->view) return ix->persistent_wave == 1;
    if (ix->persistent_wave >= 0) return ix->persistent_wave != 0;
    return ix->ws.B >= 2048 && ix->ws.W * ix->avg_degree0 <= 24.0;
}

template <bool L2, bool F16, class GA>
static int launch_persist_nch(lm_index* ix, const PersistArgs& a, const GA& g, size_t shmem) {
    dim3 grid(ix->ws.B);
    const bool wave = persist_wave_form(ix);
    switch (ix->Dp / 64) {
#define CASEP(n)                                                                                                         \
    case n:                                                                                                              \
        if (wave) {                                                                                                      \
            LM_HIP(hipFuncSetAttribute((const void*)k_search_table<n, L2, F16, 64, GA>, hipFuncAttributeMaxDynamicSharedMemorySize, (int)shmem)); \
            hipLaunchKernelGGL((k_search_table<n, L2, F16, 64, GA>), grid, dim3(64), shmem, ix->stream, g, ix->ws, a);        \
        } else {                                                                                                         \
            LM_HIP(hipFuncSetAttribute((const void*)k_search_table<n, L2, F16, 256, GA>, hipFuncAttributeMaxDynamicSharedMemorySize, (int)shmem)); \
            hipLaunchKernelGGL((k_search_table<n, L2, F16, 256, GA>), grid, dim3(256), shmem, ix->stream, g, ix->ws, a);      \
        }                                                                                                                \
        break
        CASEP(1); CASEP(2); CASEP(3); CASEP(4); CASEP(5); CASEP(6); CASEP(8); CASEP(12); CASEP(16);
#undef CASEP
        default: LM_FAIL(LM_EINVAL, "unsupported padded dimension (supported: 64..384, 512, 768, 1024)");
    }
    LM_HIP(hipGetLastError());
    return LM_OK;
}

#define VIEW_LDS_TEXT "efSearch / k / beam_size too large for a view index: (2*max(efSearch,k) + P(maxnew)) * 8 + 4 * maxnew bytes, maxnew = max(beam_size * levels[0].cap, largest upper cap, 1), must fit 150 KiB"

#define LOCKSTEP_LDS_TEXT "efSearch / beam_size / batch_size too large for the LDS-resident pool (2*max(efSearch,k) + max(beam*max_degree, batch_size + max_degree) keys must fit 64 KiB)"

static int view_checks(const lm_index* ix, int64_t n, int32_t k, const lm_search_params* prm) {
    if (!ix || !ix->view || !prm || n <= 0 || k <= 0 || prm->efSearch <= 0 || prm->batch_size < 0) return LM_OK;
    if (prm->recompute) LM_FAIL(LM_ESTATE, "a view index searches stored embeddings only: recompute = 1 is not served (lm_index_create_view)");
    if (prm->batch_size > 0) LM_FAIL(LM_ESTATE, "a view index has no dynamic batching: batch_size > 0 is not served (lm_index_create_view)");
    if (prm->pq_pruning_ratio > 0.0f) LM_FAIL(LM_ESTATE, "a view index has no two-level search: pq_pruning_ratio > 0 is not served (lm_index_create_view)");
    if (!ix->persistent_table) LM_FAIL(LM_ESTATE, "a view index has no lock-step search: option persistent_table = 0 is not served (lm_index_create_view)");
    if (ix->N == 0) return LM_OK;
    if (!ix->d_table) LM_FAIL(LM_ESTATE, "a view index needs a stored-embedding table (lm_index_attach_table)");
    const int64_t W = std::max(prm->beam_size, 1);
    if (W > 64) LM_FAIL(LM_EINVAL, "beam_size > 64 is not supported by the persistent search kernel, the only one a view index has");
    const int64_t maxnew = std::max<int64_t>({W * ix->maxdeg0, (int64_t)ix->maxdeg_up, (int64_t)1});
    int64_t P = 1;
    while (P < maxnew) P <<= 1;
    if ((2 * (int64_t)std::max(prm->efSearch, k) + P) * 8 + 4 * maxnew > 150 * 1024) LM_FAIL(LM_EINVAL, VIEW_LDS_TEXT);
    return LM_OK;
}

static int search_pass_persistent(lm_index* ix, int32_t B, const float* d_q, int32_t k, const lm_search_params& prm,
                                  float* d_dist, int64_t* d_labels) {
    const int32_t ef = std::max(prm.efSearch, k);
    const int32_t W = std::max(prm.beam_size, 1);
    int rc = ensure_ws(ix, B, ef, W);
    if (rc) return rc;
    WsDev& ws = ix->ws;
    ws.efs = prm.efSearch;
    ws.batch = 0;
    ws.check_rel = prm.check_relative_distance;
    hipStream_t st = ix->stream;
    if ((rc = ensure_pq_counters(ix, B)) != LM_OK) return rc;
    PersistArgs a{};
    a.Q = d_q; a.E = ix->d_table; a.check_rel = prm.check_relative_distance; a.max_level = ix->max_level;
    a.Pmax = next_pow2(ws.maxnew); a.k = k; a.metric = ix->metric; a.labels = d_labels; a.dist = d_dist;
    a.rounds_q = ix->d_pq_rounds.get();
    const size_t shmem = ((size_t)2 * ef + a.Pmax) * 8 + (size_t)ws.maxnew * 4;
    if (shmem > 150 * 1024) {
        if (ix->view) LM_FAIL(LM_EINVAL, VIEW_LDS_TEXT);
        return 1;
    }
    LM_HIP(hipMemsetAsync(ws.visited, 0, (size_t)B * ws.nw * 4, st));
    LM_HIP(hipMemsetAsync(ws.counters, 0, C_NCOUNTERS * sizeof(unsigned long long), st));
    {
        EvScope es(ix, &ix->ev_update);
        const bool f16 = ix->table_dtype == LM_DTYPE_F16, l2 = ix->metric == LM_METRIC_L2;
        auto go = [&](const auto& g) {
            return l2 ? (f16 ? launch_persist_nch<true, true>(ix, a, g, shmem) : launch_persist_nch<true, false>(ix, a, g, shmem))
                      : (f16 ? launch_persist_nch<false, true>(ix, a, g, shmem) : launch_persist_nch<false, false>(ix, a, g, shmem));
        };
        if (ix->view) rc = go(ViewDev{ix->N, ix->entry_point, ix->max_level, ix->view_levels[0].d_adj, ix->view_levels[0].cap, ix->d_view_up.get()});
        else rc = go(GraphDev{ix->N, ix->entry_point, ix->max_level, ix->d_node_offsets.get(), ix->d_level_ptr.get(), ix->d_neighbors.get(), ix->d_l0.get()});
    }
    if (rc) return rc;
    ix->stats.update_launches++;
    hipLaunchKernelGGL(k_stats, dim3(1), dim3(256), 0, st, ws);
    hipLaunchKernelGGL(k_rounds_max, dim3(1), dim3(256), 0, st, ws, ix->d_pq_rounds.get());
    unsigned long long* hc = ix->h_counters;
    LM_HIP(hipMemcpyAsync(hc, ws.counters, C_NCOUNTERS * sizeof(unsigned long long), hipMemcpyDeviceToHost, st));
    LM_HIP(hipStreamSynchronize(st));
    ix->stats.nrounds = std::max<int64_t>(ix->stats.nrounds, (int64_t)hc[C_ROUNDS]);
    ix->stats.ndis += (int64_t)hc[C_NDIS];
    ix->stats.nexpand += (int64_t)hc[C_NEXPAND];
    return LM_OK;
}

static int search_pass(lm_index* ix, int32_t B, const float* d_q, int32_t k, const lm_search_params& prm,
                       float* d_dist, int64_t* d_labels, const FilterPass* flt = nullptr) {
    const int32_t ef = std::max(prm.efSearch, k);
    const int32_t W = std::max(prm.beam_size, 1);
    const bool prune = prm.pq_pruning_ratio > 0.0f;
    if (prune) {
        if (!ix->d_pq_codes.get()) LM_FAIL(LM_ESTATE, "pq_pruning_ratio > 0 needs a product quantiser (lm_pq_attach)");
        if (prm.pq_pruning_ratio >= 1.0f) LM_FAIL(LM_EINVAL, "pq_pruning_ratio must be < 1");
    }
    const bool recompute = prm.recompute != 0;
    const int spec = (recompute && prm.recompute_memo != 0 && !prune && B <= ix->speculate_max_batch) ? ix->speculate : 0;
    int rc = ensure_ws(ix, B, ef, W, prune, spec, prm.batch_size);
    if (rc) return rc;
    WsDev& ws = ix->ws;
    ws.efs = prm.efSearch;
    ws.batch = prm.batch_size;
    ws.check_rel = prm.check_relative_distance;
    hipStream_t st = ix->stream;
    PruneArgs pa{};
    size_t prune_shmem = 0;
    if (prune) {
        if ((rc = ix->d_lut.reserve((size_t)B * ix->pq_m * 256)) != LM_OK) return rc;
        pa.Q = d_q; pa.lut = ix->d_lut.get(); pa.codebooks = ix->d_pq_codebooks.get(); pa.codes = ix->d_pq_codes.get();
        pa.Dp = ix->Dp; pa.metric = ix->metric; pa.m = ix->pq_m; pa.chunk_off = ix->d_pq_chunk_off.get();
        pa.keep = 1.0f - prm.pq_pruning_ratio;
        pa.strategy = prm.local_prune ? 1 : (prm.send_neigh_times_ratio > 1e-6f ? 2 : 0);
        pa.Pmax = next_pow2(ws.maxnew);
        prune_shmem = ((size_t)pa.Pmax + 2 * AQ_CAP) * 8;
        hipLaunchKernelGGL(k_pq_lut_all, dim3(B), dim3(256), 0, st, pa);
    }
    const bool hub = recompute && ix->hub_n > 0;
    const bool memo_call = recompute && prm.recompute_memo != 0 && (B > 1 || spec > 0);
    const bool memo = memo_call || hub;
    int64_t memo_used = 0;
    if (memo) {
        if ((rc = ix->d_memo_slot.reserve((size_t)ix->N)) != LM_OK) return rc;
        const int64_t first = ix->memo_initial_rows > 0 ? ix->memo_initial_rows : std::max<int64_t>(65536, (int64_t)B * 1024);
        if ((rc = ensure_memo_rows(ix, std::min<int64_t>(ix->N, ix->hub_n + (memo_call ? first : 0)), hub ? ix->hub_n : 0)) != LM_OK) return rc;
        ws.memo_slot = ix->d_memo_slot.get();
        ws.memo = ix->d_memo;
        if (hub) {
            LM_HIP(hipMemcpyAsync(ix->d_memo_slot.get(), ix->d_hub_slot_init.get(), (size_t)ix->N * 4, hipMemcpyDeviceToDevice, st));
            memo_used = ix->hub_n;
        } else {
            LM_HIP(hipMemsetAsync(ix->d_memo_slot.get(), 0xFF, (size_t)ix->N * 4, st));
        }
    }
    GraphDev g{ix->N, ix->entry_point, ix->max_level, ix->d_node_offsets.get(), ix->d_level_ptr.get(), ix->d_neighbors.get(), ix->d_l0.get()};
    const bool single = recompute && B == 1 && !memo && !prune && ix->single_query_direct != 0;

    LM_HIP(hipMemsetAsync(ws.visited, 0, (size_t)B * ws.nw * 4, st));
    LM_HIP(hipMemsetAsync(ws.counters, 0, C_NCOUNTERS * sizeof(unsigned long long), st));
    hipLaunchKernelGGL(k_init, dim3((B + 255) / 256), dim3(256), 0, st, ws, ix->max_level);
    FilterDev fd{};
    if (flt) {
        if ((rc = ensure_filter_ws(ix, B, k, fd)) != LM_OK) return rc;
        fd.allow = flt->d_allow;
        hipLaunchKernelGGL(k_filter_init, dim3((B + 255) / 256), dim3(256), 0, st, fd, B);
    }

    UpdateArgs ua{};
    unsigned long long* span_acc = nullptr;
    if (ix->profiling) {
        if ((rc = ix->d_tstamp.reserve((size_t)2 * B + 2)) != LM_OK) return rc;
        ua.tstamp = ix->d_tstamp.get();
        span_acc = ix->d_tstamp.get() + ix->d_tstamp.capacity() - 2;
        LM_HIP(hipMemsetAsync(ix->d_tstamp.get(), 0, ix->d_tstamp.capacity() * 8, st));
    }
    ua.Q = d_q;
    ua.check_rel = prm.check_relative_distance;
    ua.max_level = ix->max_level;
    {
        const size_t need = ((size_t)2 * ef + next_pow2(ws.maxnew)) * 8;
        if (need > 64 * 1024) LM_FAIL(LM_EINVAL, LOCKSTEP_LDS_TEXT);
    }
    const int ntiles = (int)((ws.nw + UNIQ_TILE - 1) / UNIQ_TILE);
    const int sync_every = recompute ? 1 : 4;
    int64_t rounds = 0;
    unsigned long long* hc = ix->h_counters;

    const int32_t* round_ids = single ? ws.newid : ws.uniq;
    ua.identity = single ? 1 : 0;
    for (;;) {
        if (!single) LM_HIP(hipMemsetAsync(ws.counters + C_LIVE, 0, sizeof(unsigned long long), st));
        {
            EvScope es(ix, &ix->ev_expand);
            hipLaunchKernelGGL(k_expand, dim3(B), dim3(64), (size_t)ws.maxnew * sizeof(int32_t), st, g, ws, single ? 0 : recompute ? (memo ? 2 : 1) : 0,
                               (int)(rounds + 1), prune ? 1 : 0, single ? 1 : 0);
            if (prune) {
                pa.use_rbm = recompute ? (memo ? 2 : 1) : 0;
                hipLaunchKernelGGL(k_prune, dim3(B), dim3(256), prune_shmem, st, ws, pa);
            }
            if (spec > 0) hipLaunchKernelGGL(k_speculate, dim3(B), dim3(64), 0, st, g, ws, spec, (int)prm.check_relative_distance);
            if (recompute && !single) {
                hipLaunchKernelGGL(k_uniq_count, dim3(ntiles), dim3(256), 0, st, ws);
                hipLaunchKernelGGL(k_uniq_emit, dim3(ntiles), dim3(256), 0, st, ws, ntiles);
            }
        }
        rounds++;
        const bool native = recompute && ix->native_rc && ix->provider == lm_recompute_provider && ix->provider_user == (void*)ix->native_rc;
        if (native && (rc = rc_prepare(ix->native_rc, round_ids, ws.counters + C_NUNIQ, single ? (int64_t)ws.maxnew : ix->ws_ucap, ws.counters + C_RC_TOKENS,
                                       ws.counters + C_RC_MAXLEN, st)) != LM_OK)
            return rc;
        bool do_sync = (rounds % sync_every) == 0;
        if (do_sync) {
            LM_HIP(hipMemcpyAsync(hc, ws.counters, C_NCOUNTERS * sizeof(unsigned long long), hipMemcpyDeviceToHost, st));
            LM_HIP(hipStreamSynchronize(st));
            if (hc[C_LIVE] == 0) break;
        }
        if (recompute) {
            int32_t nu = (int32_t)hc[C_NUNIQ];
            void* d_e = nullptr;
            ix->stats.nunique += nu;
            if (native) rc_prepared(ix->native_rc, round_ids, nu, (int64_t)hc[C_RC_TOKENS], (int32_t)hc[C_RC_MAXLEN]);
            if (nu > 0) {
                EvScope es(ix, &ix->ev_provider);
                int prc = ix->provider(ix->provider_user, round_ids, nu, &d_e, (void*)st);
                if (prc != 0 || !d_e) LM_FAIL(LM_EPROVIDER, "embedding provider failed (rc=" + std::to_string(prc) + ")");
            }
            if (memo) {
                if (nu > 0) {
                    if ((rc = ensure_memo_rows(ix, memo_used + nu, memo_used)) != LM_OK) return rc;
                    hipLaunchKernelGGL(k_memo_append, dim3((unsigned)std::min<int64_t>(2048, ((int64_t)nu * (ix->Dp / 4) + 255) / 256)),
                                       dim3(256), 0, st, ws, (const float*)d_e, nu, memo_used, ix->Dp);
                    if (memo_call) memo_used += nu;
                }
                ua.E = ix->d_memo;
                ua.by_rank = 2;
            } else {
                ua.E = d_e;
                ua.by_rank = 1;
            }
            if (flt && (rc = launch_filter_collect(ix, ua, false, fd)) != LM_OK) return rc;
            EvScope es(ix, &ix->ev_update);
            rc = launch_update(ix, ua, false);
        } else {
            ua.E = ix->d_table;
            ua.by_rank = 0;
            if (flt && (rc = launch_filter_collect(ix, ua, ix->table_dtype == LM_DTYPE_F16, fd)) != LM_OK) return rc;
            EvScope es(ix, &ix->ev_update);
            rc = launch_update(ix, ua, ix->table_dtype == LM_DTYPE_F16);
        }
        if (rc) return rc;
        if (hub && !memo_call && recompute && hc[C_NUNIQ] > 0)
            hipLaunchKernelGGL(k_memo_release, dim3((unsigned)std::min<int64_t>(1024, ((int64_t)hc[C_NUNIQ] + 255) / 256)), dim3(256), 0, st, ws,
                               (int32_t)hc[C_NUNIQ]);
        if (span_acc) hipLaunchKernelGGL(k_span, dim3(1), dim3(256), 0, st, ix->d_tstamp.get(), B, span_acc);
        ix->stats.update_launches++;
    }
    if (flt) {
        hipLaunchKernelGGL(k_filter_finalize, dim3((B * k + 255) / 256), dim3(256), 0, st, fd, B, ix->metric, d_labels, d_dist);
        hipLaunchKernelGGL(k_filter_total, dim3(1), dim3(256), 0, st, fd, B);
    } else {
        hipLaunchKernelGGL(k_finalize, dim3((B * k + 255) / 256), dim3(256), 0, st, ws, k, ix->metric, d_labels, d_dist);
    }
    hipLaunchKernelGGL(k_stats, dim3(1), dim3(256), 0, st, ws);
    LM_HIP(hipGetLastError());
    LM_HIP(hipMemcpyAsync(hc, ws.counters, C_NCOUNTERS * sizeof(unsigned long long), hipMemcpyDeviceToHost, st));
    LM_HIP(hipStreamSynchronize(st));
    if (flt) {
        unsigned long long total = 0;
        LM_HIP(hipMemcpy(&total, fd.nallow + B, sizeof(total), hipMemcpyDeviceToHost));
        ix->filtered_allowed_evals += (int64_t)total;
    }
    if (flt && flt->rounds_max) ix->stats.nrounds = std::max<int64_t>(ix->stats.nrounds, (int64_t)hc[C_ROUNDS]);
    else ix->stats.nrounds += (int64_t)hc[C_ROUNDS];
    ix->stats.ndis += (int64_t)hc[C_NDIS];
    ix->stats.nexpand += (int64_t)hc[C_NEXPAND];
    ix->stats.nadc += (int64_t)hc[C_NADC];
    if (span_acc) {
        unsigned long long acc[2] = {0, 0};
        LM_HIP(hipMemcpy(acc, span_acc, sizeof(acc), hipMemcpyDeviceToHost));
        int khz = 100000;
        (void)hipDeviceGetAttribute(&khz, hipDeviceAttributeWallClockRate, ix->device);
        ix->span_ms += (double)acc[0] / (double)khz;
        ix->span_launches += (int64_t)acc[1];
    }
    return LM_OK;
}

static int search_lds_checks(const lm_index* ix, int32_t k, const lm_search_params& prm, bool persistent, bool* fits_persistent) {
    const int64_t ef = std::max(prm.efSearch, k), W = std::max(prm.beam_size, 1);
    const int64_t maxnew = ws_maxnew(ix, W, prm.pq_pruning_ratio > 0.0f, prm.batch_size);
    const int64_t keys = 2 * ef + next_pow2_64(maxnew);
    *fits_persistent = persistent && keys * 8 + 4 * maxnew <= 150 * 1024;
    if (!*fits_persistent && keys * 8 > 64 * 1024) LM_FAIL(LM_EINVAL, LOCKSTEP_LDS_TEXT);
    return LM_OK;
}

static int do_search_device(lm_index* ix, int64_t n, const float* d_x, int32_t k, float* d_dist, int64_t* d_labels,
                            const lm_search_params* params, const FilterPass* flt = nullptr) {
    if (!ix || !params || n < 0 || k <= 0) LM_FAIL(LM_EINVAL, "bad search arguments");
    lm_search_params prm = *params;
    if (prm.efSearch <= 0) LM_FAIL(LM_EINVAL, "efSearch must be positive");
    if (prm.batch_size < 0) LM_FAIL(LM_EINVAL, "batch_size must not be negative (0 = no dynamic batching)");
    if (int vrc = view_checks(ix, n, k, &prm)) return vrc;
    LM_HIP(hipSetDevice(ix->device));
    if (flt) ix->filtered_allowed_evals = 0;
    ix->stats = lm_search_stats{};
    ix->span_ms = 0;
    ix->span_launches = 0;
    (void)drain_events(ix, ix->ev_update);
    (void)drain_events(ix, ix->ev_expand);
    (void)drain_events(ix, ix->ev_provider);
    if (n == 0) return LM_OK;
    hipStream_t st = ix->stream;
    if (ix->N == 0 || ix->entry_point < 0) {
        hipLaunchKernelGGL(k_fill_empty, dim3((unsigned)((n * k + 255) / 256)), dim3(256), 0, st, n * (int64_t)k,
                           ix->metric, d_labels, d_dist);
        LM_HIP(hipStreamSynchronize(st));
        return LM_OK;
    }
    if (prm.recompute) {
        if (!ix->provider) LM_FAIL(LM_ESTATE, "recompute requested but no embedding provider is attached");
    } else if (!ix->d_table) {
        LM_FAIL(LM_ESTATE, "index stores no embeddings (pruned): recompute is required");
    }
    const bool persistent = ix->view || (!prm.recompute && prm.pq_pruning_ratio <= 0.0f && prm.batch_size == 0 && ix->persistent_table &&
                                         ix->update_variant == 0 && std::max(prm.beam_size, 1) <= 64);
    bool fits_persistent = ix->view;
    if (!ix->view)
        if (int lrc = search_lds_checks(ix, k, prm, persistent && !flt, &fits_persistent)) return lrc;
    const float* d_q = nullptr;
    if (int prc = pad_queries(ix, n, d_x, &d_q)) return prc;
    int64_t maxb = prm.max_batch > 0 ? prm.max_batch : 4096;
    int64_t nwbytes = ((ix->N + 31) / 32) * 4;
    maxb = std::max<int64_t>(1, std::min<int64_t>(maxb, (8ll << 30) / std::max<int64_t>(nwbytes, 1)));
    FilterPass fpass{};
    if (flt) {
        bool unfiltered_persistent = false;
        if (int lrc = search_lds_checks(ix, k, prm, persistent, &unfiltered_persistent)) return lrc;
        fpass = *flt;
        fpass.rounds_max = unfiltered_persistent;
        flt = &fpass;
    }
    for (int64_t off = 0; off < n; off += maxb) {
        int32_t B = (int32_t)std::min<int64_t>(maxb, n - off);
        int rc = 1;
        if (!flt && fits_persistent)
            rc = search_pass_persistent(ix, B, d_q + (size_t)off * ix->Dp, k, prm, d_dist + (size_t)off * k, d_labels + (size_t)off * k);
        if (rc == 1 && ix->view) LM_FAIL(LM_ESTATE, "internal: a view index has no lock-step search");
        if (rc == 1)
            rc = search_pass(ix, B, d_q + (size_t)off * ix->Dp, k, prm, d_dist + (size_t)off * k, d_labels + (size_t)off * k, flt);
        if (rc) return rc;
    }
    LM_HIP(hipStreamSynchronize(st));
    if (ix->profiling) {
        ix->stats.update_ms = drain_events(ix, ix->ev_update);
        ix->stats.expand_ms = drain_events(ix, ix->ev_expand);
        ix->stats.provider_ms = drain_events(ix, ix->ev_provider);
        ix->stats.update_span_ms = ix->span_ms;
        ix->stats.update_span_launches = ix->span_launches;
        if (ix->span_launches == 0) {
            ix->stats.update_span_ms = ix->stats.update_ms;
            ix->stats.update_span_launches = ix->stats.update_launches;
        }
    }
    return LM_OK;
}

static void compute_degrees(lm_index* ix, const uint64_t* node_offsets, const uint64_t* level_ptr, std::vector<L0Range>& l0) {
    int32_t m0 = 0, mu = 0;
    l0.resize((size_t)ix->N);
    for (int64_t i = 0; i < ix->N; ++i) {
        uint64_t p0 = node_offsets[i], p1 = node_offsets[i + 1];
        l0[i] = L0Range{p1 > p0 + 1 ? level_ptr[p0] : 0, p1 > p0 + 1 ? (uint32_t)(level_ptr[p0 + 1] - level_ptr[p0]) : 0u, 0u};
        for (uint64_t p = p0; p + 1 < p1; ++p) {
            int32_t deg = (int32_t)(level_ptr[p + 1] - level_ptr[p]);
            if (p == p0) m0 = std::max(m0, deg);
            else mu = std::max(mu, deg);
        }
    }
    ix->maxdeg0 = m0;
    ix->maxdeg_up = mu;
    double e0 = 0;
    for (int64_t i = 0; i < ix->N; ++i) e0 += l0[i].count;
    ix->avg_degree0 = ix->N ? e0 / (double)ix->N : 0.0;
}

extern "C" {

const char* lm_last_error(void) { return g_err.c_str(); }
const char* lm_version(void) { return "leann-mi355x 0.2 (gfx950)"; }
int lm_abi_revision(void) { return LM_ABI_REVISION; }

int lm_device_count(void) {
    int n = 0;
    if (hipGetDeviceCount(&n) != hipSuccess) return 0;
    return n;
}

void lm_search_params_default(lm_search_params* p) {
    if (!p) return;
    std::memset(p, 0, sizeof(*p));
    p->efSearch = 64;
    p->beam_size = 1;
    p->check_relative_distance = 1;
    p->recompute = 1;
    p->max_batch = 0;
    p->recompute_memo = 1;
}

int lm_index_create_from_csr(int64_t ntotal, int32_t d, int32_t metric, const uint64_t* node_offsets,
                             const uint64_t* level_ptr, int64_t n_level_ptr, const int32_t* neighbors,
                             int64_t n_neighbors, const int32_t* levels, int32_t entry_point, int32_t max_level,
                             int device, lm_index** out) {
    if (!out) LM_FAIL(LM_EINVAL, "out is NULL");
    *out = nullptr;
    if (ntotal < 0 || d <= 0 || (metric != LM_METRIC_L2 && metric != LM_METRIC_INNER_PRODUCT))
        LM_FAIL(LM_EINVAL, "bad ntotal / d / metric");
    if (ntotal > 0 && (!node_offsets || !level_ptr || !levels)) LM_FAIL(LM_EINVAL, "NULL CSR array");
    if (ntotal > 0x7fffffff) LM_FAIL(LM_EINVAL, "ntotal exceeds int32 node ids");
    if (ntotal > 0) {
        if ((int64_t)node_offsets[ntotal] != n_level_ptr) LM_FAIL(LM_EFORMAT, "node_offsets[ntotal] != len(level_ptr)");
        if (entry_point < 0 || entry_point >= ntotal) LM_FAIL(LM_EFORMAT, "entry_point out of range");
        if (levels[entry_point] != max_level + 1) LM_FAIL(LM_EFORMAT, "levels[entry_point] != max_level + 1");
        for (int64_t i = 0; i < ntotal; ++i)
            if ((int64_t)(node_offsets[i + 1] - node_offsets[i]) != (int64_t)levels[i] + 1)
                LM_FAIL(LM_EFORMAT, "node_offsets[i+1]-node_offsets[i] != levels[i]+1");
        for (int64_t p = 0; p + 1 < n_level_ptr; ++p)
            if (level_ptr[p + 1] < level_ptr[p]) LM_FAIL(LM_EFORMAT, "level_ptr not monotone");
        if (n_level_ptr > 0 && (int64_t)level_ptr[n_level_ptr - 1] > n_neighbors) LM_FAIL(LM_EFORMAT, "level_ptr past neighbors");
        for (int64_t e = 0; e < n_neighbors; ++e)
            if (neighbors[e] < 0 || neighbors[e] >= ntotal) LM_FAIL(LM_EFORMAT, "neighbor id out of range");
    }
    int ndev = lm_device_count();
    if (ndev <= 0) LM_FAIL(LM_EHIP, "no HIP device visible: libleann_mi355x requires an MI355X (gfx950) GPU");
    if (device < 0 || device >= ndev) LM_FAIL(LM_EINVAL, "device index out of range");
    LM_HIP(hipSetDevice(device));
    lm_index* ix = new lm_index();
    ix->device = device;
    ix->N = ntotal; ix->D = d; ix->Dp = (d + 63) / 64 * 64; ix->metric = metric;
    ix->entry_point = ntotal > 0 ? entry_point : -1;
    ix->max_level = max_level;
    ix->n_neighbors = n_neighbors; ix->n_level_ptr = n_level_ptr;
    if (ntotal > 0) {
        std::vector<L0Range> l0;
        compute_degrees(ix, node_offsets, level_ptr, l0);
        hipError_t e = hipSuccess;
        if (ix->d_l0.reserve((size_t)ntotal) || ix->d_node_offsets.reserve((size_t)ntotal + 1) || ix->d_level_ptr.reserve((size_t)n_level_ptr) ||
            ix->d_neighbors.reserve((size_t)n_neighbors)) {
            lm_index_free(ix);
            return LM_EHIP;
        }
        if ((e = hipMemcpy(ix->d_l0.get(), l0.data(), (size_t)ntotal * sizeof(L0Range), hipMemcpyHostToDevice)) != hipSuccess ||
            (e = hipMemcpy(ix->d_node_offsets.get(), node_offsets, (size_t)(ntotal + 1) * 8, hipMemcpyHostToDevice)) != hipSuccess ||
            (e = hipMemcpy(ix->d_level_ptr.get(), level_ptr, (size_t)n_level_ptr * 8, hipMemcpyHostToDevice)) != hipSuccess ||
            (e = hipMemcpy(ix->d_neighbors.get(), neighbors, (size_t)n_neighbors * 4, hipMemcpyHostToDevice)) != hipSuccess) {
            set_error(std::string("graph upload failed: ") + hipGetErrorString(e));
            lm_index_free(ix);
            return LM_EHIP;
        }
    }
    if (hipHostMalloc((void**)&ix->h_counters, C_NCOUNTERS * sizeof(unsigned long long)) != hipSuccess) {
        set_error("hipHostMalloc failed");
        lm_index_free(ix);
        return LM_EHIP;
    }
    std::memset(ix->h_counters, 0, C_NCOUNTERS * sizeof(unsigned long long));
    *out = ix;
    return LM_OK;
}

int lm_index_read(const char* path, int device, lm_index** out) {
    if (!out || !path) LM_FAIL(LM_EINVAL, "NULL argument");
    *out = nullptr;
    HostCsr h;
    int rc = read_csr_file(path, h);
    if (rc) return rc;
    rc = lm_index_create_from_csr(h.ntotal, h.d, h.metric, h.node_offsets.data(), h.level_ptr.data(),
                                  (int64_t)h.level_ptr.size(), h.neighbors.data(), (int64_t)h.neighbors.size(),
                                  h.levels.data(), h.entry_point, h.max_level, device, out);
    if (rc) return rc;
    if (!h.storage.empty()) {
        rc = lm_index_attach_table(*out, h.storage.data(), LM_DTYPE_F32, h.ntotal, h.d, 0);
        if (rc) {
            lm_index_free(*out);
            *out = nullptr;
        }
    }
    return rc;
}

int lm_index_create_view(int64_t ntotal, int32_t d, int32_t metric, const lm_graph_level* levels, int32_t n_levels, int32_t entry_point, int device,
                         lm_index** out) {
    if (!out) LM_FAIL(LM_EINVAL, "out is NULL");
    *out = nullptr;
    if (!levels) LM_FAIL(LM_EINVAL, "levels is NULL");
    if (n_levels < 1) LM_FAIL(LM_EINVAL, "n_levels must be at least 1");
    if (ntotal < 0 || ntotal > 0x7fffffffll) LM_FAIL(LM_EINVAL, "ntotal must be in [0, INT32_MAX]");
    if (metric != LM_METRIC_L2 && metric != LM_METRIC_INNER_PRODUCT) LM_FAIL(LM_EINVAL, "unknown metric");
    if (d <= 0 || d > 1024) LM_FAIL(LM_EINVAL, "unsupported dimension (padded to a multiple of 64: 64..384, 512, 768, 1024)");
    switch ((d + 63) / 64) {
        case 1: case 2: case 3: case 4: case 5: case 6: case 8: case 12: case 16: break;
        default: LM_FAIL(LM_EINVAL, "unsupported dimension (padded to a multiple of 64: 64..384, 512, 768, 1024)");
    }
    int64_t nn = 0;
    int32_t cap_up = 0;
    for (int32_t l = 0; l < n_levels; ++l) {
        const lm_graph_level& L = levels[l];
        const std::string at = "levels[" + std::to_string(l) + "]: ";
        if (L.cap < 1) LM_FAIL(LM_EINVAL, at + "cap must be at least 1");
        if (L.n_rows < 0 || L.n_rows > ntotal) LM_FAIL(LM_EINVAL, at + "n_rows must be in [0, ntotal]");
        if (l == 0 && (L.d_nodes || L.n_rows != ntotal)) LM_FAIL(LM_EINVAL, "levels[0] must be the identity level: d_nodes NULL and n_rows == ntotal");
        if (l > 0 && L.n_rows > 0 && !L.d_nodes && L.n_rows != ntotal) LM_FAIL(LM_EINVAL, at + "d_nodes is NULL but n_rows != ntotal");
        if (L.n_rows > 0 && !L.d_adj) LM_FAIL(LM_EINVAL, at + "d_adj is NULL");
        nn += L.n_rows * (int64_t)L.cap;
        if (l > 0) cap_up = std::max(cap_up, L.cap);
    }
    if (ntotal > 0 && (entry_point < 0 || entry_point >= ntotal)) LM_FAIL(LM_EINVAL, "entry_point out of range");
    int ndev = lm_device_count();
    if (ndev <= 0) LM_FAIL(LM_EHIP, "no HIP device visible: libleann_mi355x requires an MI355X (gfx950) GPU");
    if (device < 0 || device >= ndev) LM_FAIL(LM_EINVAL, "device index out of range");
    LM_HIP(hipSetDevice(device));
    lm_index* ix = new lm_index();
    ix->device = device;
    ix->view = true;
    ix->view_levels.assign(levels, levels + n_levels);
    ix->N = ntotal; ix->D = d; ix->Dp = (d + 63) / 64 * 64; ix->metric = metric;
    ix->entry_point = ntotal > 0 ? entry_point : -1;
    ix->max_level = n_levels - 1;
    ix->maxdeg0 = levels[0].cap;
    ix->maxdeg_up = cap_up;
    ix->n_neighbors = nn;
    std::vector<ViewLevelDev> up;
    for (int32_t l = 1; l < n_levels; ++l) up.push_back(ViewLevelDev{levels[l].d_nodes, levels[l].d_adj, (int32_t)levels[l].n_rows, levels[l].cap});
    hipError_t e = hipSuccess;
    if (!up.empty() && ix->d_view_up.reserve(up.size())) {
        lm_index_free(ix);
        return LM_EHIP;
    }
    if (!up.empty() && (e = hipMemcpy(ix->d_view_up.get(), up.data(), up.size() * sizeof(ViewLevelDev), hipMemcpyHostToDevice)) != hipSuccess) {
        set_error(std::string("level descriptor upload failed: ") + hipGetErrorString(e));
        lm_index_free(ix);
        return LM_EHIP;
    }
    if (hipHostMalloc((void**)&ix->h_counters, C_NCOUNTERS * sizeof(unsigned long long)) != hipSuccess) {
        set_error("hipHostMalloc failed");
        lm_index_free(ix);
        return LM_EHIP;
    }
    std::memset(ix->h_counters, 0, C_NCOUNTERS * sizeof(unsigned long long));
    *out = ix;
    return LM_OK;
}

void lm_index_free(lm_index* ix) {
    if (!ix) return;
    (void)hipSetDevice(ix->device);
    free_ws(ix);
    if (ix->d_memo) (void)hipFree(ix->d_memo);
    if (ix->d_table && ix->table_owned) (void)hipFree(ix->d_table);
    (void)drain_events(ix, ix->ev_update);
    (void)drain_events(ix, ix->ev_expand);
    (void)drain_events(ix, ix->ev_provider);
    for (hipEvent_t e : ix->ev_pool) (void)hipEventDestroy(e);
    if (ix->h_counters) (void)hipHostFree(ix->h_counters);
    delete ix;
}

int lm_index_info(const lm_index* ix, lm_index_info_t* o) {
    if (!ix || !o) LM_FAIL(LM_EINVAL, "NULL argument");
    o->ntotal = ix->N; o->d = ix->D; o->d_padded = ix->Dp; o->metric = ix->metric;
    o->entry_point = ix->entry_point; o->max_level = ix->max_level;
    o->max_degree0 = ix->maxdeg0; o->max_degree_up = ix->maxdeg_up; o->n_neighbors = ix->n_neighbors;
    o->has_table = ix->d_table != nullptr; o->has_provider = ix->provider != nullptr; o->device = ix->device;
    return LM_OK;
}

int lm_index_attach_table(lm_index* ix, const void* table, int32_t dtype, int64_t ntotal, int32_t d, int32_t location) {
    if (!ix || !table) LM_FAIL(LM_EINVAL, "NULL argument");
    if (ntotal != ix->N || d != ix->D) LM_FAIL(LM_EINVAL, "table shape does not match the index");
    if (dtype != LM_DTYPE_F32 && dtype != LM_DTYPE_F16) LM_FAIL(LM_EINVAL, "dtype must be f32 or f16");
    LM_HIP(hipSetDevice(ix->device));
    if (ix->d_table && ix->table_owned) (void)hipFree(ix->d_table);
    ix->d_table = nullptr;
    ix->table_owned = false;
    ix->table_dtype = dtype;
    if (location == 1) {
        ix->d_table = const_cast<void*>(table);
        return LM_OK;
    }
    size_t es = dtype == LM_DTYPE_F16 ? 2 : 4;
    void* dst = nullptr;
    LM_HIP(hipMalloc(&dst, std::max<size_t>((size_t)ntotal * ix->Dp * es, 16)));
    ix->d_table = dst;
    ix->table_owned = true;
    if (ix->D == ix->Dp) {
        LM_HIP(hipMemcpy(dst, table, (size_t)ntotal * d * es, hipMemcpyHostToDevice));
    } else {
        void* tmp = nullptr;
        LM_HIP(hipMalloc(&tmp, std::max<size_t>((size_t)ntotal * d * es, 16)));
        if (hipMemcpy(tmp, table, (size_t)ntotal * d * es, hipMemcpyHostToDevice) != hipSuccess) {
            (void)hipFree(tmp);
            LM_FAIL(LM_EHIP, "table upload failed");
        }
        int64_t tot = ntotal * ix->Dp;
        if (dtype == LM_DTYPE_F32)
            hipLaunchKernelGGL(k_pad_rows, dim3((unsigned)((tot + 255) / 256)), dim3(256), 0, 0, (const float*)tmp, ntotal, d, ix->Dp, (float*)dst);
        else
            hipLaunchKernelGGL(k_pad_rows_f16, dim3((unsigned)((tot + 255) / 256)), dim3(256), 0, 0, (const __half*)tmp, ntotal, d, ix->Dp, (__half*)dst);
        const hipError_t pe = hipDeviceSynchronize();
        (void)hipFree(tmp);
        LM_HIP(pe);
    }
    return LM_OK;
}

int lm_index_set_hub_cache(lm_index* ix, const int32_t* ids, int32_t n, const float* d_embeddings) {
    if (!ix) LM_FAIL(LM_EINVAL, "NULL index");
    LM_NOT_ON_VIEW(ix, "lm_index_set_hub_cache");
    LM_HIP(hipSetDevice(ix->device));
    if (n == 0) {
        ix->hub_n = 0;
        return LM_OK;
    }
    if (n < 0 || !ids || !d_embeddings || n > ix->N) LM_FAIL(LM_EINVAL, "bad hub cache arguments");
    std::vector<int32_t> slot((size_t)ix->N, -1);
    for (int32_t i = 0; i < n; ++i) {
        if (ids[i] < 0 || ids[i] >= ix->N || slot[ids[i]] >= 0) LM_FAIL(LM_EINVAL, "hub ids must be unique and in range");
        slot[ids[i]] = i;
    }
    if (int mrc = ensure_memo_rows(ix, n, 0)) return mrc;
    if (int hrc = ix->d_hub_slot_init.reserve((size_t)ix->N)) return hrc;
    LM_HIP(hipMemcpy(ix->d_hub_slot_init.get(), slot.data(), (size_t)ix->N * 4, hipMemcpyHostToDevice));
    LM_HIP(hipMemcpy(ix->d_memo, d_embeddings, (size_t)n * ix->Dp * 4, hipMemcpyDeviceToDevice));
    ix->hub_n = n;
    return LM_OK;
}

int lm_index_set_provider(lm_index* ix, lm_provider_fn fn, void* user) {
    if (!ix) LM_FAIL(LM_EINVAL, "NULL index");
    ix->provider = fn;
    ix->provider_user = user;
    return LM_OK;
}

int lm_index_set_recompute(lm_index* ix, lm_recompute* rc) {
    if (!ix) LM_FAIL(LM_EINVAL, "NULL index");
    if (rc && ix->Dp != lm::rc_width(rc))
        LM_FAIL(LM_EINVAL, "lm_index_set_recompute: the provider's embeddings are " + std::to_string(lm::rc_width(rc)) + " wide; this index has padded d = " +
                               std::to_string(ix->Dp));
    ix->native_rc = rc;
    ix->provider = rc ? lm_recompute_provider : nullptr;
    ix->provider_user = rc;
    return LM_OK;
}

int lm_index_set_stream(lm_index* ix, void* s) {
    if (!ix) LM_FAIL(LM_EINVAL, "NULL index");
    ix->stream = (hipStream_t)s;
    return LM_OK;
}

int lm_index_set_profiling(lm_index* ix, int32_t enable) {
    if (!ix) LM_FAIL(LM_EINVAL, "NULL index");
    ix->profiling = enable != 0;
    return LM_OK;
}

int lm_index_set_option(lm_index* ix, const char* name, int64_t value) {
    if (!ix || !name) LM_FAIL(LM_EINVAL, "NULL argument");
    if (!std::strcmp(name, "update_variant")) {
        if (value != 0 && value != 3 && value != 4)
            LM_FAIL(LM_EINVAL, "update_variant must be 0 (auto), 3 (wave per query) or 4 (workgroup per query); 1 and 2 were removed");
        ix->update_variant = (int)value;
        return LM_OK;
    }
    if (!std::strcmp(name, "persistent_table")) {
        ix->persistent_table = value != 0;
        return LM_OK;
    }
    if (!std::strcmp(name, "pq_threads")) {
        if (value != 256 && value != 512 && value != 1024) LM_FAIL(LM_EINVAL, "pq_threads must be 256, 512 or 1024");
        ix->pq_threads = (int)value;
        return LM_OK;
    }
    if (!std::strcmp(name, "pq_rerank_expanded")) {
        ix->pq_rerank_expanded = value != 0;
        ix->pq_overflow = 0;
        return LM_OK;
    }
    if (!std::strcmp(name, "persistent_wave")) {
        if (value < -1 || value > 1) LM_FAIL(LM_EINVAL, "persistent_wave must be -1 (auto), 0 or 1");
        ix->persistent_wave = (int)value;
        return LM_OK;
    }
    if (!std::strcmp(name, "wave_maxnew")) {
        ix->wave_maxnew = (int)value;
        return LM_OK;
    }
    if (!std::strcmp(name, "single_query_direct")) {
        ix->single_query_direct = value != 0;
        return LM_OK;
    }
    if (!std::strcmp(name, "speculate")) {
        if (value < 0 || value > 64) LM_FAIL(LM_EINVAL, "speculate must be in [0, 64]");
        ix->speculate = (int)value;
        return LM_OK;
    }
    if (!std::strcmp(name, "speculate_max_batch")) {
        if (value < 1) LM_FAIL(LM_EINVAL, "speculate_max_batch must be >= 1");
        ix->speculate_max_batch = (int)std::min<int64_t>(value, 1 << 20);
        return LM_OK;
    }
    if (!std::strcmp(name, "memo_initial_rows")) {
        if (value < 0) LM_FAIL(LM_EINVAL, "memo_initial_rows must not be negative");
        ix->memo_initial_rows = value;
        return LM_OK;
    }
    LM_FAIL(LM_EINVAL, std::string("unknown option: ") + name);
}

int lm_index_get_option(const lm_index* ix, const char* name, int64_t* value) {
    if (!ix || !name || !value) LM_FAIL(LM_EINVAL, "NULL argument");
    if (!std::strcmp(name, "pq_rerank_overflow")) *value = ix->pq_overflow;
    else if (!std::strcmp(name, "pq_rerank_expanded")) *value = ix->pq_rerank_expanded ? 1 : 0;
    else if (!std::strcmp(name, "pq_threads")) *value = ix->pq_threads;
    else if (!std::strcmp(name, "speculate")) *value = ix->speculate;
    else if (!std::strcmp(name, "single_query_direct")) *value = ix->single_query_direct;
    else if (!std::strcmp(name, "speculate_max_batch")) *value = ix->speculate_max_batch;
    else if (!std::strcmp(name, "filtered_allowed_evals")) *value = ix->filtered_allowed_evals;
    else LM_FAIL(LM_EINVAL, std::string("unknown readable option: ") + name);
    return LM_OK;
}

int lm_index_event_overhead_us(lm_index* ix, double* out_us) {
    if (!ix || !out_us) LM_FAIL(LM_EINVAL, "NULL argument");
    LM_HIP(hipSetDevice(ix->device));
    const int reps = 256;
    std::vector<std::pair<hipEvent_t, hipEvent_t>> ev(reps);
    int64_t* dl = nullptr;
    float* dd = nullptr;
    LM_HIP(hipMalloc((void**)&dl, 64));
    LM_HIP(hipMalloc((void**)&dd, 64));
    for (int w = 0; w < 2; ++w) {
        for (int i = 0; i < reps; ++i) {
            if (w == 0) {
                (void)hipEventCreate(&ev[i].first);
                (void)hipEventCreate(&ev[i].second);
            }
            (void)hipEventRecord(ev[i].first, ix->stream);
            hipLaunchKernelGGL(k_fill_empty, dim3(1), dim3(64), 0, ix->stream, (int64_t)0, 0, dl, dd);
            (void)hipEventRecord(ev[i].second, ix->stream);
        }
        LM_HIP(hipStreamSynchronize(ix->stream));
    }
    double ms = 0;
    for (auto& p : ev) {
        float t = 0;
        (void)hipEventElapsedTime(&t, p.first, p.second);
        ms += t;
        (void)hipEventDestroy(p.first);
        (void)hipEventDestroy(p.second);
    }
    (void)hipFree(dl);
    (void)hipFree(dd);
    *out_us = 1e3 * ms / reps;
    return LM_OK;
}

int lm_index_get_stats(const lm_index* ix, lm_search_stats* out) {
    if (!ix || !out) LM_FAIL(LM_EINVAL, "NULL argument");
    *out = ix->stats;
    return LM_OK;
}

int lm_index_search_device(lm_index* ix, int64_t n, const float* d_x, int32_t k, float* d_distances, int64_t* d_labels,
                           const lm_search_params* params) {
    if (n > 0 && (!d_x || !d_distances || !d_labels)) LM_FAIL(LM_EINVAL, "NULL buffer");
    return do_search_device(ix, n, d_x, k, d_distances, d_labels, params);
}

int lm_index_search(lm_index* ix, int64_t n, const float* x, int32_t k, float* distances, int64_t* labels,
                    const lm_search_params* params) {
    if (!ix) LM_FAIL(LM_EINVAL, "NULL index");
    if (n < 0 || k <= 0) LM_FAIL(LM_EINVAL, "bad n / k");
    if (n == 0) return LM_OK;
    if (!x || !distances || !labels) LM_FAIL(LM_EINVAL, "NULL buffer");
    if (int vrc = view_checks(ix, n, k, params)) return vrc;
    LM_HIP(hipSetDevice(ix->device));
    if (int rc = stage_in(ix, x, n, k)) return rc;
    if (int rc = do_search_device(ix, n, ix->d_stage_x.get(), k, ix->d_stage_d.get(), ix->d_stage_l.get(), params)) return rc;
    return stage_out(ix, distances, labels, n, k);
}

static int filtered_checks(const lm_index* ix, int64_t n, int32_t k, const lm_search_params* params) {
    if (!ix || !params || n < 0 || k <= 0) LM_FAIL(LM_EINVAL, "bad search arguments");
    if (params->efSearch <= 0) LM_FAIL(LM_EINVAL, "efSearch must be positive");
    if (params->batch_size < 0) LM_FAIL(LM_EINVAL, "batch_size must not be negative (0 = no dynamic batching)");
    if (params->pq_pruning_ratio > 0.0f)
        LM_FAIL(LM_EINVAL, "the filtered graph search takes no pq_pruning_ratio: the two-level search does not evaluate every new node exactly");
    if (n == 0 || ix->N == 0 || ix->entry_point < 0) return LM_OK;
    if (params->recompute) {
        if (!ix->provider) LM_FAIL(LM_ESTATE, "recompute requested but no embedding provider is attached");
    } else if (!ix->d_table) {
        LM_FAIL(LM_ESTATE, "index stores no embeddings (pruned): recompute is required");
    }
    return LM_OK;
}

int lm_index_search_filtered_device(lm_index* ix, int64_t n, const float* d_x, int32_t k, const uint32_t* d_allow, float* d_distances,
                                    int64_t* d_labels, const lm_search_params* params) {
    LM_NOT_ON_VIEW(ix, "lm_index_search_filtered_device");
    if (int rc = filtered_checks(ix, n, k, params)) return rc;
    if (n > 0 && (!d_x || !d_distances || !d_labels)) LM_FAIL(LM_EINVAL, "NULL buffer");
    const FilterPass flt{d_allow};
    return do_search_device(ix, n, d_x, k, d_distances, d_labels, params, &flt);
}

int lm_index_search_filtered(lm_index* ix, int64_t n, const float* x, int32_t k, const uint32_t* allow, float* distances, int64_t* labels,
                             const lm_search_params* params) {
    LM_NOT_ON_VIEW(ix, "lm_index_search_filtered");
    if (int rc = filtered_checks(ix, n, k, params)) return rc;
    FilterPass flt{nullptr};
    if (n == 0) return do_search_device(ix, 0, nullptr, k, nullptr, nullptr, params, &flt);
    if (!x || !distances || !labels) LM_FAIL(LM_EINVAL, "NULL buffer");
    LM_HIP(hipSetDevice(ix->device));
    if (int rc = upload_allow(ix, allow, &flt.d_allow)) return rc;
    if (int rc = stage_in(ix, x, n, k)) return rc;
    if (int rc = do_search_device(ix, n, ix->d_stage_x.get(), k, ix->d_stage_d.get(), ix->d_stage_l.get(), params, &flt)) return rc;
    return stage_out(ix, distances, labels, n, k);
}

int lm_dist_gather(const void* d_table, int32_t dtype, int32_t d_padded, int32_t metric, const float* d_q,
                   const int32_t* d_qidx, const int32_t* d_ids, int64_t npairs, float* d_out, void* stream) {
    if (npairs == 0) return LM_OK;
    if (!d_table || !d_q || !d_qidx || !d_ids || !d_out) LM_FAIL(LM_EINVAL, "NULL buffer");
    if (d_padded <= 0 || d_padded % 64) LM_FAIL(LM_EINVAL, "d_padded must be a positive multiple of 64");
    dim3 grid((unsigned)((npairs + 15) / 16)), block(256);
    hipStream_t st = (hipStream_t)stream;
    const bool l2 = metric == LM_METRIC_L2, f16 = dtype == LM_DTYPE_F16;
#define GO(n)                                                                                                     \
    case n:                                                                                                       \
        if (l2 && f16) hipLaunchKernelGGL((k_dist_pairs<n, true, true>), grid, block, 0, st, d_table, d_q, d_qidx, d_ids, npairs, d_out);        \
        else if (l2) hipLaunchKernelGGL((k_dist_pairs<n, true, false>), grid, block, 0, st, d_table, d_q, d_qidx, d_ids, npairs, d_out);         \
        else if (f16) hipLaunchKernelGGL((k_dist_pairs<n, false, true>), grid, block, 0, st, d_table, d_q, d_qidx, d_ids, npairs, d_out);        \
        else hipLaunchKernelGGL((k_dist_pairs<n, false, false>), grid, block, 0, st, d_table, d_q, d_qidx, d_ids, npairs, d_out);                \
        break
    switch (d_padded / 64) {
        GO(1); GO(2); GO(3); GO(4); GO(5); GO(6); GO(8); GO(12); GO(16);
        default: LM_FAIL(LM_EINVAL, "unsupported padded dimension");
    }
#undef GO
    LM_HIP(hipGetLastError());
    return LM_OK;
}

int lm_topk_merge(const int64_t* d_in_ids, const float* d_in_dist, int32_t S, int32_t B, int32_t k, int32_t metric,
                  int64_t* d_out_ids, float* d_out_dist, void* stream) {
    if (B == 0) return LM_OK;
    if (!d_in_ids || !d_in_dist || !d_out_ids || !d_out_dist || S <= 0 || k <= 0) LM_FAIL(LM_EINVAL, "bad merge arguments");
    int P2 = next_pow2(S * k);
    if (P2 > 2048) LM_FAIL(LM_EINVAL, "S*k too large for the merge kernel (<= 2048)");
    hipLaunchKernelGGL(k_topk_merge, dim3(B), dim3(64), (size_t)P2 * 16, (hipStream_t)stream, d_in_ids, d_in_dist, S, B, k,
                       metric, P2, d_out_ids, d_out_dist);
    LM_HIP(hipGetLastError());
    return LM_OK;
}

}

#include "lm_pq_impl.h"
#include "lm_select_impl.h"
#include "lm_pq_build_impl.h"
#include "lm_exact_impl.h"
#include "lm_pq_flat_impl.h"
#include "lm_link_impl.h"
#include "lm_prune_impl.h"
#include "lm_insert_impl.h"
```

### leann_amd/csrc/lm_timing.cpp

```cpp
#include <algorithm>
#include <atomic>
#include <deque>
#include <map>
#include <mutex>
#include <vector>

#include "lm_internal.h"

namespace lm {
namespace {
struct Pair {
    hipEvent_t a, b;
    int kid, dev;
    double work;
    void* stream;
};
struct Acc {
    int64_t launches = 0;
    double ms = 0, work = 0;
};
struct DevState {
    std::vector<hipEvent_t> free_events;
    hipEvent_t last_end = nullptr;
    void* last_stream = nullptr;
    unsigned long long* d_attn_work = nullptr;
};
std::atomic<unsigned> g_mask{0};
std::mutex g_mu;
std::deque<Pair> g_pending;
std::map<int, DevState> g_dev;
Acc g_acc[LM_KT_COUNT];
const char* const g_names[LM_KT_COUNT] = {"lm::k_layer_tail_h384", "lm::k_gemm_ws_h384", "lm::k_attn_varlen", "lm::k_gemm_f16", "lm::k_qkv_h384",
                                         "lm::k_qkv_attn_h384"};

int current_device() {
    int d = 0;
    if (hipGetDevice(&d) != hipSuccess) (void)hipGetLastError();
    return d;
}
hipEvent_t get_event(int dev) {
    auto& fr = g_dev[dev].free_events;
    if (!fr.empty()) {
        hipEvent_t e = fr.back();
        fr.pop_back();
        return e;
    }
    hipEvent_t e = nullptr;
    if (hipEventCreate(&e) == hipSuccess) return e;
    (void)hipGetLastError();
    return nullptr;
}
void fold(const Pair& p) {
    DevState& ds = g_dev[p.dev];
    float ms = 0.f;
    if (hipEventElapsedTime(&ms, p.a, p.b) == hipSuccess) {
        float over = 0.f;
        if (ds.last_end && ds.last_stream == p.stream && hipEventElapsedTime(&over, p.a, ds.last_end) == hipSuccess && over > 0.f) ms -= std::min(over, ms);
        (void)hipGetLastError();
        g_acc[p.kid].launches += 1;
        g_acc[p.kid].ms += ms;
        g_acc[p.kid].work += p.work;
    } else {
        (void)hipGetLastError();
    }
    ds.free_events.push_back(p.a);
    if (ds.last_end) ds.free_events.push_back(ds.last_end);
    ds.last_end = p.b;
    ds.last_stream = p.stream;
}

__global__ __launch_bounds__(256) void k_kt_attn_work(const int32_t* __restrict__ cu, int32_t n_seqs, unsigned long long hidden,
                                                      unsigned long long* __restrict__ acc) {
    __shared__ unsigned long long s_part[4];
    unsigned long long v = 0;
    for (int i = threadIdx.x; i < n_seqs; i += 256) {
        const unsigned long long len = (unsigned long long)(cu[i + 1] - cu[i]);
        v += len * len;
    }
    for (int d = 32; d >= 1; d >>= 1) v += __shfl_xor(v, d);
    if ((threadIdx.x & 63) == 0) s_part[threadIdx.x >> 6] = v;
    __syncthreads();
    if (threadIdx.x == 0) atomicAdd(acc, (s_part[0] + s_part[1] + s_part[2] + s_part[3]) * hidden);
}
}

KtScope::KtScope(int kid_, void* stream, double work_) : kid(kid_), st(stream), work(work_), a(nullptr), dev(0) {
    if (!(g_mask.load(std::memory_order_relaxed) & (1u << kid))) return;
    std::lock_guard<std::mutex> lk(g_mu);
    while (!g_pending.empty() && hipEventQuery(g_pending.front().b) == hipSuccess) {
        fold(g_pending.front());
        g_pending.pop_front();
    }
    (void)hipGetLastError();
    dev = current_device();
    hipEvent_t e = get_event(dev);
    if (e && hipEventRecord(e, (hipStream_t)st) == hipSuccess) a = e;
    else if (e) {
        (void)hipGetLastError();
        g_dev[dev].free_events.push_back(e);
    }
}
KtScope::~KtScope() {
    if (!a) return;
    std::lock_guard<std::mutex> lk(g_mu);
    hipEvent_t b = get_event(dev);
    if (b && hipEventRecord(b, (hipStream_t)st) == hipSuccess) g_pending.push_back(Pair{(hipEvent_t)a, b, kid, dev, work, st});
    else {
        (void)hipGetLastError();
        g_dev[dev].free_events.push_back((hipEvent_t)a);
        if (b) g_dev[dev].free_events.push_back(b);
    }
}

void kt_attn_work(const int32_t* d_cu_seqlens, int32_t n_seqs, int32_t hidden, void* stream, int kid) {
    if (!(g_mask.load(std::memory_order_relaxed) & (1u << kid))) return;
    unsigned long long* acc;
    {
        std::lock_guard<std::mutex> lk(g_mu);
        DevState& ds = g_dev[current_device()];
        if (!ds.d_attn_work) {
            if (hipMalloc((void**)&ds.d_attn_work, 16) != hipSuccess || hipMemset(ds.d_attn_work, 0, 16) != hipSuccess) {
                (void)hipGetLastError();
                ds.d_attn_work = nullptr;
                return;
            }
        }
        acc = ds.d_attn_work + (kid == LM_KT_QKV_ATTN ? 1 : 0);
    }
    hipLaunchKernelGGL(k_kt_attn_work, dim3(1), dim3(256), 0, (hipStream_t)stream, d_cu_seqlens, n_seqs, (unsigned long long)hidden, acc);
    (void)hipGetLastError();
}
}

extern "C" int lm_kernel_timing_enable(uint32_t mask) {
    lm::g_mask.store(mask & ((1u << LM_KT_COUNT) - 1), std::memory_order_relaxed);
    return LM_OK;
}

extern "C" int lm_kernel_timing_read(lm_kernel_time* out, int32_t capacity, int32_t reset) {
    using namespace lm;
    if (!out || capacity < 0) LM_FAIL(LM_EINVAL, "lm_kernel_timing_read: NULL argument / negative capacity");
    std::lock_guard<std::mutex> lk(g_mu);
    while (!g_pending.empty()) {
        (void)hipEventSynchronize(g_pending.front().b);
        fold(g_pending.front());
        g_pending.pop_front();
    }
    const int before = current_device();
    for (auto& kv : g_dev) {
        if (!kv.second.d_attn_work) continue;
        unsigned long long h[2] = {0, 0};
        if (hipSetDevice(kv.first) == hipSuccess && hipMemcpy(h, kv.second.d_attn_work, 16, hipMemcpyDeviceToHost) == hipSuccess) {
            g_acc[LM_KT_ATTN].work += 4.0 * (double)h[0];
            g_acc[LM_KT_QKV_ATTN].work += 4.0 * (double)h[1];
            (void)hipMemset(kv.second.d_attn_work, 0, 16);
        } else {
            (void)hipGetLastError();
        }
    }
    (void)hipSetDevice(before);
    for (int i = 0; i < LM_KT_COUNT; ++i) {
        if (i < capacity) {
            out[i].name = g_names[i];
            out[i].launches = g_acc[i].launches;
            out[i].ms = g_acc[i].ms;
            out[i].work = g_acc[i].work;
        }
        if (reset) g_acc[i] = Acc{};
    }
    return LM_OK;
}
```

### leann_amd/recompute.py

```python

from __future__ import annotations

import ctypes as C
import os

import torch

from .encoder import BertEncoder
from .token_store import TokenStore


class RecomputeProvider:

    def __init__(self, encoder: BertEncoder, tokens: TokenStore, d_padded: int, device: torch.device,
                 batch_size: int = 5461, bucket: int = 32, max_seq_length: int | None = None):
        self.encoder = encoder
        self.tokens = tokens
        self.dp = d_padded
        self.device = device
        self.batch_size = batch_size
        self.bucket = bucket
        self.T = min(max_seq_length or encoder.cfg.max_seq_length, encoder.cfg.max_pos, max(tokens.max_len, 1))
        self._cap = 0
        self._ids = self._lens = self._out = None
        self._chunks = 0
        self._native_chunks0 = 0
        self.tokens_seen = 0
        self.count_tokens = False
        self._native = None
        self._native_tried = False
        import weakref

        self._attached = weakref.WeakSet()

    def native(self):
        from .encoder import KERNEL_SELECTION_KEYS, KernelTimers

        if (os.environ.get("LEANN_MI355X_NATIVE_PROVIDER", "1") != "1" or os.environ.get("LEANN_MI355X_ONECALL", "1") != "1"
                or KernelTimers.active is not None or any(k in os.environ for k in KERNEL_SELECTION_KEYS)):
            return None
        cfg = self.encoder.cfg
        fused = cfg.hidden == 384 and self.T <= 256
        pk = self.encoder.onecall_model() if fused else None
        if pk is None:
            fused, pk = False, self.encoder.general_model()
        if self._native_tried and pk is getattr(self, "_native_pack", None):
            return self._native
        self.close()
        self._native_tried, self._native_pack = True, pk
        t_max = 256 if cfg.heads and cfg.hidden == cfg.heads * 32 else 512
        if pk is None or not (0 < self.T <= t_max) or self.dp != cfg.hidden or not self.encoder.word.weight.is_cuda:
            return None
        from . import _lib

        h = C.c_void_p()
        create = _lib.load().lm_recompute_create if fused else _lib.load().lm_recompute_create_general
        _lib.check(create(C.byref(pk["model"]), self.tokens._h, int(self.T), int(self.batch_size) * 192, C.byref(h)),
                   "lm_recompute_create" if fused else "lm_recompute_create_general")
        self._native = h
        return h

    def native_stats(self) -> dict:
        from . import _lib

        st = _lib.RecomputeStats()
        if self._native is not None:
            _lib.check(_lib.load().lm_recompute_get_stats(self._native, C.byref(st)), "lm_recompute_get_stats")
        return {n: int(getattr(st, n)) for n, _ in _lib.RecomputeStats._fields_}

    @property
    def chunks(self) -> int:
        return self._chunks + (self.native_stats()["chunks"] - self._native_chunks0 if self._native is not None else 0)

    @chunks.setter
    def chunks(self, v: int) -> None:
        self._chunks = int(v)
        self._native_chunks0 = self.native_stats()["chunks"] if self._native is not None else 0

    def close(self) -> None:
        if self._native is not None:
            from . import _lib

            for idx in list(self._attached):
                if getattr(idx, "_h", None) and getattr(idx, "native_provider", False) and idx._provider_keepalive is self:
                    idx.set_provider(None)
            self._attached.clear()
            _lib.load().lm_recompute_free(self._native)
            self._native = None
        self._native_tried = False

    def __del__(self):
        try:
            self.close()
        except Exception:
            pass

    def _ensure(self, n: int):
        if n > self._cap:
            cap = max(n, int(self._cap * 1.5), 1024)
            self._ids = torch.empty((cap, self.T), dtype=torch.int32, device=self.device)
            self._lens = torch.empty((cap,), dtype=torch.int32, device=self.device)
            self._out = torch.zeros((cap, self.dp), dtype=torch.float32, device=self.device)
            self._cap = cap

    @torch.no_grad()
    def __call__(self, d_ids_ptr: int, n: int, stream_ptr: int) -> int:
        self._ensure(n)
        ids, lens = self._ids[:n], self._lens[:n]
        self.tokens.gather(d_ids_ptr, n, self.T, self.encoder.cfg.pad_id, ids, lens, stream_ptr)
        emb = self.encoder.encode_tokens(ids, lens, batch_size=self.batch_size, bucket=self.bucket)
        d = emb.shape[1]
        if d == self.dp:
            self._keep = emb.contiguous()
            out = self._keep
        else:
            self._out[:n, :d] = emb
            out = self._out
        self._chunks += n
        if self.count_tokens:
            self.tokens_seen += int(lens.sum())
        return out.data_ptr()

    @torch.no_grad()
    def embed_ids(self, ids: torch.Tensor) -> torch.Tensor:
        n = ids.shape[0]
        stream = torch.cuda.current_stream(self.device).cuda_stream
        h = self.native()
        if h is not None and ids.dtype == torch.int32 and ids.is_contiguous():
            from . import _lib

            out = torch.empty((n, self.encoder.cfg.hidden), dtype=torch.float32, device=ids.device)
            _lib.check(_lib.load().lm_recompute_embed(h, C.c_void_p(ids.data_ptr()), n, C.c_void_p(out.data_ptr()), C.c_void_p(stream)),
                       "lm_recompute_embed")
            return out
        self._ensure(n)
        self.tokens.gather(ids.data_ptr(), n, self.T, self.encoder.cfg.pad_id, self._ids[:n], self._lens[:n], stream)
        return self.encoder.encode_tokens(self._ids[:n], self._lens[:n], batch_size=self.batch_size, bucket=self.bucket)
```

Baseline: 661.1.

## Split large recompute forwards into token-balanced parts on parallel HIP streams

The recompute provider now splits one large packed BERT forward into up to three token-balanced parts. The length-scan kernel computes the split points on the device, and each part runs on its own lane stream, forked and joined with events and given its own token and workspace buffers. The aim is to overlap several smaller forwards and so fill the GPU better than one serial forward. The cost is extra stream and event management, duplicated workspace memory, and a per-part forward plan that must stay on the large-forward kernels. It also adds lanes options and reworks kernel-timing overlap accounting for multiple streams.

```diff
diff --git a/include/leann_mi355x.h b/include/leann_mi355x.h
--- a/include/leann_mi355x.h
+++ b/include/leann_mi355x.h
@@ -295,6 +295,8 @@
                      int32_t *d_out_ids, int32_t *d_out_len, void *stream);
 int64_t lm_tokens_count(const lm_tokens *t);
 
+#define LM_RC_LANE_MIN_TOKENS LM_BERT_QKV_GEMM_TOKENS
+#define LM_RC_DEFAULT_LANES 3
 typedef struct lm_recompute lm_recompute;
 typedef struct lm_recompute_stats {
     int64_t calls, chunks, tokens, forwards, host_syncs;
@@ -307,6 +309,8 @@
 int lm_recompute_provider(void *user, const int32_t *d_ids, int32_t n, void **d_out, void *stream);
 int lm_recompute_embed(lm_recompute *rc, const int32_t *d_ids, int32_t n, float *d_out, void *stream);
 int lm_recompute_get_stats(const lm_recompute *rc, lm_recompute_stats *out);
+int lm_recompute_set_option(lm_recompute *rc, const char *name, int64_t value);
+int lm_recompute_get_option(const lm_recompute *rc, const char *name, int64_t *out);
 int lm_index_set_recompute(lm_index *idx, lm_recompute *rc);
 
 #define LM_KT_LAYER_TAIL 0
diff --git a/leann_amd/_lib.py b/leann_amd/_lib.py
--- a/leann_amd/_lib.py
+++ b/leann_amd/_lib.py
@@ -117,7 +117,7 @@
     "lm_tokens_create", "lm_tokens_free", "lm_tokens_gather", "lm_tokens_count",
     "lm_bert_h384_workspace_bytes", "lm_bert_h384_forward_packed",
     "lm_bert_workspace_bytes", "lm_bert_forward_packed", "lm_clspool_varlen_f16",
-    "lm_recompute_create", "lm_recompute_create_general", "lm_recompute_free", "lm_recompute_provider", "lm_recompute_embed", "lm_recompute_get_stats", "lm_index_set_recompute",
+    "lm_recompute_create", "lm_recompute_create_general", "lm_recompute_free", "lm_recompute_provider", "lm_recompute_embed", "lm_recompute_get_stats", "lm_recompute_set_option", "lm_recompute_get_option", "lm_index_set_recompute",
     "lm_kernel_timing_enable", "lm_kernel_timing_read",
 ]
 
@@ -228,6 +228,8 @@
     lib.lm_recompute_provider.argtypes = [vp, vp, i32, C.POINTER(vp), vp]
     lib.lm_recompute_embed.argtypes = [vp, vp, i32, vp, vp]
     lib.lm_recompute_get_stats.argtypes = [vp, C.POINTER(RecomputeStats)]
+    lib.lm_recompute_set_option.argtypes = [vp, C.c_char_p, i64]
+    lib.lm_recompute_get_option.argtypes = [vp, C.c_char_p, C.POINTER(C.c_int64)]
     lib.lm_index_set_recompute.argtypes = [vp, vp]
     lib.lm_kernel_timing_enable.argtypes = [C.c_uint32]
     lib.lm_kernel_timing_read.argtypes = [C.POINTER(KernelTime), i32, i32]
diff --git a/leann_amd/csrc/lm_device_types.h b/leann_amd/csrc/lm_device_types.h
--- a/leann_amd/csrc/lm_device_types.h
+++ b/leann_amd/csrc/lm_device_types.h
@@ -47,7 +47,7 @@
     float* memo;
     unsigned long long* counters;
 };
-enum { C_LIVE = 0, C_NUNIQ = 1, C_NDIS = 2, C_NEXPAND = 3, C_ROUNDS = 4, C_RC_TOKENS = 5, C_NADC = 6, C_RC_MAXLEN = 7, C_PQ_OVERFLOW = 8, C_PQ_ALLOWED = 9, C_NCOUNTERS = 10 };
+enum { C_LIVE = 0, C_NUNIQ = 1, C_NDIS = 2, C_NEXPAND = 3, C_ROUNDS = 4, C_RC_TOKENS = 5, C_NADC = 6, C_RC_MAXLEN = 7, C_PQ_OVERFLOW = 8, C_PQ_ALLOWED = 9, C_RC_SPLIT = 10, C_NCOUNTERS = 12 };
 
 constexpr int UNIQ_TILE = 4096;
 constexpr int AQ_CAP = 512;
diff --git a/leann_amd/csrc/lm_encoder_forward.cpp b/leann_amd/csrc/lm_encoder_forward.cpp
--- a/leann_amd/csrc/lm_encoder_forward.cpp
+++ b/leann_amd/csrc/lm_encoder_forward.cpp
@@ -37,10 +37,28 @@
     return (size_t)total_tokens * (3 * 384 + 1152) * 2 + small;
 }
 
+lm::BertH384Plan lm::bert_h384_plan(const lm_bert_h384* m, int32_t n_seqs, int64_t total_tokens, int32_t max_len) {
+    BertH384Plan p;
+    p.small = total_tokens <= small_tokens_limit() && m->ffn % 128 == 0;
+    for (int l = 0; p.small && l < m->n_layers; ++l) p.small = m->layers[l].wo && m->layers[l].w1 && m->layers[l].w2;
+    p.first_half = h384_first_half_form(m->heads, max_len, total_tokens, n_seqs);
+    p.qkv_gemm = !p.small && total_tokens <= qkv_gemm_tokens_limit();
+    for (int l = 0; p.qkv_gemm && l < m->n_layers; ++l) p.qkv_gemm = m->layers[l].wqkv != nullptr;
+    const char* f = getenv("LEANN_MI355X_FUSED_QKV_ATTN");
+    if (p.qkv_gemm && f && f[0] == '1') p.qkv_gemm = false;
+    else if (p.qkv_gemm) p.first_half = H384_PAIR_ROW_MAJOR;
+    return p;
+}
+
 extern "C" int lm_bert_h384_forward_packed(const lm_bert_h384* m, const int32_t* d_tok, const int32_t* d_pos, const int32_t* d_cu_seqlens,
                                            int32_t n_seqs, int64_t total_tokens, int32_t max_len, void* d_workspace, size_t workspace_bytes,
                                            float* d_out, void* stream) {
-    using namespace lm;
+    return lm::bert_h384_forward_planned(m, d_tok, d_pos, d_cu_seqlens, n_seqs, total_tokens, max_len, d_workspace, workspace_bytes, d_out, nullptr, stream);
+}
+
+int lm::bert_h384_forward_planned(const lm_bert_h384* m, const int32_t* d_tok, const int32_t* d_pos, const int32_t* d_cu_seqlens, int32_t n_seqs,
+                                  int64_t total_tokens, int32_t max_len, void* d_workspace, size_t workspace_bytes, float* d_out,
+                                  const BertH384Plan* plan, void* stream) {
     if (n_seqs == 0 || total_tokens == 0) return LM_OK;
     if (!m || !m->layers || !d_tok || !d_pos || !d_cu_seqlens || !d_workspace || !d_out || n_seqs < 0 || total_tokens < 0)
         LM_FAIL(LM_EINVAL, "lm_bert_h384_forward_packed: bad arguments");
@@ -56,17 +74,12 @@
     void* qkv = ws + 3 * row;
     int rc = lm_embed_layernorm_f16(d_tok, d_pos, m->word, m->pos_table, m->type0, m->emb_gamma, m->emb_beta, x, total_tokens, 384, m->ln_eps, stream);
     if (rc) return rc;
-    bool small = total_tokens <= small_tokens_limit() && m->ffn % 128 == 0;
-    for (int l = 0; small && l < m->n_layers; ++l) small = m->layers[l].wo && m->layers[l].w1 && m->layers[l].w2;
+    const BertH384Plan pl = plan ? *plan : bert_h384_plan(m, n_seqs, total_tokens, max_len);
+    if (pl.small && total_tokens > std::max<int64_t>(small_tokens_limit(), LM_BERT_SMALL_TOKENS))
+        LM_FAIL(LM_EINVAL, "lm_bert_h384_forward_packed: a small-forward plan for a forward above the small-forward limit");
+    const bool small = pl.small, qkv_gemm = pl.qkv_gemm;
+    const H384FirstHalf first_half = pl.first_half;
     void* hid = ws + 3 * row + (size_t)total_tokens * 1152 * 2;
-    H384FirstHalf first_half = h384_first_half_form(m->heads, max_len, total_tokens, n_seqs);
-    bool qkv_gemm = !small && total_tokens <= qkv_gemm_tokens_limit();
-    for (int l = 0; qkv_gemm && l < m->n_layers; ++l) qkv_gemm = m->layers[l].wqkv != nullptr;
-    {
-        const char* f = getenv("LEANN_MI355X_FUSED_QKV_ATTN");
-        if (qkv_gemm && f && f[0] == '1') qkv_gemm = false;
-        else if (qkv_gemm) first_half = H384_PAIR_ROW_MAJOR;
-    }
     for (int l = 0; l < m->n_layers; ++l) {
         const lm_bert_h384_layer& L = m->layers[l];
         if (small) {
diff --git a/leann_amd/csrc/lm_internal.h b/leann_amd/csrc/lm_internal.h
--- a/leann_amd/csrc/lm_internal.h
+++ b/leann_amd/csrc/lm_internal.h
@@ -115,14 +115,23 @@
 struct lm_recompute;
 namespace lm {
 int rc_prepare(lm_recompute* rc, const int32_t* d_ids, const unsigned long long* d_n, int64_t cap, unsigned long long* d_total,
-               unsigned long long* d_maxlen, hipStream_t st);
-void rc_prepared(lm_recompute* rc, const int32_t* d_ids, int32_t n, int64_t total, int32_t max_len);
+               unsigned long long* d_maxlen, unsigned long long* d_split, hipStream_t st);
+void rc_prepared(lm_recompute* rc, const int32_t* d_ids, int32_t n, int64_t total, int32_t max_len, const unsigned long long* split);
 int32_t rc_width(const lm_recompute* rc);
 inline bool bert_h384_envelope_ok(int n_layers, int heads, int ffn) { return n_layers > 0 && heads * 32 == 384 && ffn >= 192 && ffn <= 1728 && ffn % 192 == 0; }
 #define LM_BERT_H384_ENVELOPE_TEXT "hidden 384 = heads x 32 and ffn a multiple of 192 in [192, 1728]"
 enum H384FirstHalf : int { H384_FUSED = 0, H384_PAIR_HEAD_MAJOR = 1, H384_PAIR_ROW_MAJOR = 2 };
 constexpr int H384_FUSED_MIN_MEAN_LEN = 216;
 H384FirstHalf h384_first_half_form(int32_t heads, int32_t max_len, int64_t total_tokens, int32_t n_seqs);
+struct BertH384Plan {
+    bool small = false;
+    bool qkv_gemm = false;
+    H384FirstHalf first_half = H384_PAIR_HEAD_MAJOR;
+};
+BertH384Plan bert_h384_plan(const lm_bert_h384* m, int32_t n_seqs, int64_t total_tokens, int32_t max_len);
+int bert_h384_forward_planned(const lm_bert_h384* m, const int32_t* d_tok, const int32_t* d_pos, const int32_t* d_cu_seqlens, int32_t n_seqs,
+                              int64_t total_tokens, int32_t max_len, void* d_workspace, size_t workspace_bytes, float* d_out, const BertH384Plan* plan,
+                              void* stream);
 
 }
 
diff --git a/leann_amd/csrc/lm_rc_parts.h b/leann_amd/csrc/lm_rc_parts.h
--- /dev/null
+++ b/leann_amd/csrc/lm_rc_parts.h
@@ -0,0 +1,50 @@
+#pragma once
+#include <cstdint>
+
+namespace lm {
+
+constexpr int RC_MAX_LANES = 3;
+
+struct RcPart {
+    int32_t b0 = 0;
+    int32_t n = 0;
+    int64_t tokens = 0;
+};
+
+inline unsigned long long rc_split_pack(int32_t index, int64_t cu_at_index) { return ((unsigned long long)(uint32_t)cu_at_index << 32) | (uint32_t)index; }
+inline int32_t rc_split_index(unsigned long long w) { return (int32_t)(uint32_t)w; }
+inline int64_t rc_split_tokens(unsigned long long w) { return (int64_t)(w >> 32); }
+
+inline void rc_split_points(const int32_t* cu, int32_t n, int lanes, unsigned long long* out ) {
+    const int64_t total = n > 0 ? (int64_t)cu[n] : 0;
+    for (int j = 1; j < lanes; ++j) {
+        const int64_t thr = (int64_t)j * total / lanes;
+        int32_t i = 0;
+        while (i < n && (int64_t)cu[i + 1] <= thr) ++i;
+        out[j - 1] = rc_split_pack(i, i < n ? (int64_t)cu[i] : total);
+    }
+}
+
+inline int rc_plan_parts(int32_t n, int64_t total, int lanes, int64_t lane_min_tokens, const unsigned long long* split, RcPart* out ) {
+    out[0].b0 = 0;
+    out[0].n = n;
+    out[0].tokens = total;
+    if (lanes < 2 || lanes > RC_MAX_LANES || n < lanes || !split || lane_min_tokens < 0 || total <= lane_min_tokens * lanes) return 1;
+    RcPart p[RC_MAX_LANES];
+    int32_t b = 0;
+    int64_t t = 0;
+    for (int j = 0; j < lanes; ++j) {
+        const int32_t e = j + 1 < lanes ? rc_split_index(split[j]) : n;
+        const int64_t te = j + 1 < lanes ? rc_split_tokens(split[j]) : total;
+        if (e <= b || e > n || te - t <= lane_min_tokens || te > total) return 1;
+        p[j].b0 = b;
+        p[j].n = e - b;
+        p[j].tokens = te - t;
+        b = e;
+        t = te;
+    }
+    for (int j = 0; j < lanes; ++j) out[j] = p[j];
+    return lanes;
+}
+
+}
diff --git a/leann_amd/csrc/lm_recompute.hip b/leann_amd/csrc/lm_recompute.hip
--- a/leann_amd/csrc/lm_recompute.hip
+++ b/leann_amd/csrc/lm_recompute.hip
@@ -5,6 +5,28 @@
 
 #include "lm_device_types.h"
 #include "lm_internal.h"
+#include "lm_rc_parts.h"
+
+static_assert(LM_RC_LANE_MIN_TOKENS >= LM_BERT_SMALL_TOKENS && LM_RC_LANE_MIN_TOKENS >= LM_BERT_QKV_GEMM_TOKENS,
+              "a part of a split forward must not fall below the thresholds of the large-forward kernels");
+
+#if defined(LM_EMULATED_DEVICE) || defined(LM_HOST_EMULATION)
+#define LM_RC_LANES 0
+#else
+#define LM_RC_LANES 1
+#endif
+
+struct lm_rc_lane {
+    hipStream_t st = nullptr;
+    hipEvent_t done = nullptr;
+    int32_t* d_cu_sub = nullptr;
+    int64_t cu_sub_cap = 0;
+    int32_t* d_tok = nullptr;
+    int64_t tok_cap = 0;
+    void* d_ws = nullptr;
+    size_t ws_bytes = 0;
+    bool busy = false;
+};
 
 struct lm_recompute {
     int device = 0;
@@ -18,12 +40,11 @@
     int32_t T = 0;
     int64_t max_tokens = 0;
     int32_t* d_cu = nullptr;
-    int32_t* d_cu_sub = nullptr;
     int64_t cu_cap = 0;
-    int32_t* d_tok = nullptr;
-    int64_t tok_cap = 0;
-    void* d_ws = nullptr;
-    size_t ws_bytes = 0;
+    lm_rc_lane lane[lm::RC_MAX_LANES];
+    int32_t lanes = 1;
+    int64_t lane_min_tokens = LM_RC_LANE_MIN_TOKENS;
+    hipEvent_t ev_fork = nullptr;
     float* d_out = nullptr;
     int64_t out_cap = 0;
     unsigned long long* d_meta = nullptr;
@@ -33,8 +54,10 @@
     int32_t prep_n = -1;
     int64_t prep_total = 0;
     int32_t prep_maxlen = 0;
+    unsigned long long prep_split[2] = {0, 0};
     bool prep_launched = false;
     int64_t chunks = 0, tokens_seen = 0, forwards = 0, calls = 0, syncs = 0;
+    int64_t parts = 0;
 };
 
 namespace lm {
@@ -42,7 +65,8 @@
 __global__ __launch_bounds__(1024) void k_rc_lengths_scan(const uint64_t* __restrict__ off, const int32_t* __restrict__ ids, int32_t n_host,
                                                           const unsigned long long* __restrict__ d_n, int64_t cap, int32_t T,
                                                           int32_t* __restrict__ cu, unsigned long long* __restrict__ out_total,
-                                                          unsigned long long* __restrict__ out_maxlen) {
+                                                          unsigned long long* __restrict__ out_maxlen, int32_t lanes,
+                                                          unsigned long long* __restrict__ out_split) {
     __shared__ int32_t s_wave[16];
     __shared__ int32_t s_max[16];
     const int tid = threadIdx.x, lane = tid & 63, wave = tid >> 6;
@@ -88,6 +112,19 @@
         *out_total = (unsigned long long)(uint32_t)carry;
         *out_maxlen = (unsigned long long)(uint32_t)m;
     }
+    if (lanes > 1) {
+        const int64_t total = carry;
+        if (tid < lanes - 1) out_split[tid] = ((unsigned long long)(uint32_t)carry << 32) | (uint32_t)n;
+        __syncthreads();
+        if (total > 0) {
+            const int64_t thr1 = total / lanes, thr2 = 2 * total / lanes;
+            for (int64_t i = tid; i < n; i += 1024) {
+                const int64_t lo = (int64_t)cu[i], hi = (int64_t)cu[i + 1];
+                if (lo <= thr1 && thr1 < hi) out_split[0] = ((unsigned long long)(uint32_t)lo << 32) | (uint32_t)i;
+                if (lanes > 2 && lo <= thr2 && thr2 < hi) out_split[1] = ((unsigned long long)(uint32_t)lo << 32) | (uint32_t)i;
+            }
+        }
+    }
 }
 
 __global__ __launch_bounds__(256) void k_rc_pack(const uint16_t* __restrict__ tok, const uint64_t* __restrict__ off,
@@ -128,81 +165,133 @@
 
 static int rc_ensure_cu(lm_recompute* rc, int64_t n, hipStream_t st) {
     int r = rc_grow(rc, &rc->d_cu, &rc->cu_cap, 2 * (n + 1), 4, st);
-    rc->d_cu_sub = rc->d_cu + rc->cu_cap / 2;
+    rc->lane[0].d_cu_sub = rc->d_cu + rc->cu_cap / 2;
     return r;
 }
 
 int rc_prepare(lm_recompute* rc, const int32_t* d_ids, const unsigned long long* d_n, int64_t cap, unsigned long long* d_total,
-               unsigned long long* d_maxlen, hipStream_t st) {
+               unsigned long long* d_maxlen, unsigned long long* d_split, hipStream_t st) {
     rc->prep_ids = nullptr;
     rc->prep_n = -1;
     rc->prep_launched = false;
     if (cap * (int64_t)rc->T > (int64_t)INT32_MAX) return LM_OK;
     int r = rc_ensure_cu(rc, cap, st);
     if (r) return r;
-    hipLaunchKernelGGL(k_rc_lengths_scan, dim3(1), dim3(1024), 0, st, rc->tokens->d_off, d_ids, 0, d_n, cap, rc->T, rc->d_cu, d_total, d_maxlen);
+    hipLaunchKernelGGL(k_rc_lengths_scan, dim3(1), dim3(1024), 0, st, rc->tokens->d_off, d_ids, 0, d_n, cap, rc->T, rc->d_cu, d_total, d_maxlen,
+                       rc->lanes, d_split);
     LM_HIP(hipGetLastError());
     rc->prep_launched = true;
     return LM_OK;
 }
 
-void rc_prepared(lm_recompute* rc, const int32_t* d_ids, int32_t n, int64_t total, int32_t max_len) {
+void rc_prepared(lm_recompute* rc, const int32_t* d_ids, int32_t n, int64_t total, int32_t max_len, const unsigned long long* split) {
     if (!rc->prep_launched) return;
     rc->prep_launched = false;
     rc->prep_ids = d_ids;
     rc->prep_n = n;
     rc->prep_total = total;
     rc->prep_maxlen = max_len;
-}
-
-static int rc_forward(lm_recompute* rc, const int32_t* d_ids, int32_t b0, int32_t n_sub, int64_t total, int32_t max_len, float* d_out,
-                      hipStream_t st) {
+    rc->prep_split[0] = split[0];
+    rc->prep_split[1] = split[1];
+}
+
+static int rc_forward(lm_recompute* rc, int L, const int32_t* d_ids, int32_t b0, int32_t n_sub, int64_t total, int32_t max_len, float* d_out,
+                      const BertH384Plan* plan, hipStream_t caller) {
     int r;
-    if ((r = rc_grow(rc, &rc->d_tok, &rc->tok_cap, 2 * total, 4, st, (int64_t)1 << 18))) return r;
-    int32_t* d_pos = rc->d_tok + rc->tok_cap / 2;
+    lm_rc_lane& ln = rc->lane[L];
+    hipStream_t st = caller;
+#if LM_RC_LANES
+    if (L > 0) {
+        st = ln.st;
+        if (!ln.busy) {
+            LM_HIP(hipStreamWaitEvent(st, rc->ev_fork, 0));
+            ln.busy = true;
+        }
+        if ((r = rc_grow(rc, &ln.d_cu_sub, &ln.cu_sub_cap, (int64_t)n_sub + 1, 4, st))) return r;
+    }
+#endif
+    if ((r = rc_grow(rc, &ln.d_tok, &ln.tok_cap, 2 * total, 4, st, (int64_t)1 << 18))) return r;
+    int32_t* d_pos = ln.d_tok + ln.tok_cap / 2;
     const size_t need = rc->general ? lm_bert_workspace_bytes(&rc->gmodel, total) : lm_bert_h384_workspace_bytes(total);
-    if (need > rc->ws_bytes) {
-        if (rc->d_ws) {
+    if (need > ln.ws_bytes) {
+        if (ln.d_ws) {
             LM_HIP(hipStreamSynchronize(st));
             rc->syncs++;
-            (void)hipFree(rc->d_ws);
-            rc->d_ws = nullptr;
-            rc->ws_bytes = 0;
+            (void)hipFree(ln.d_ws);
+            ln.d_ws = nullptr;
+            ln.ws_bytes = 0;
         }
         const size_t want = std::max<size_t>(need + need / 4, (size_t)64 << 20);
-        LM_HIP(hipMalloc(&rc->d_ws, want));
-        rc->ws_bytes = want;
+        LM_HIP(hipMalloc(&ln.d_ws, want));
+        ln.ws_bytes = want;
     }
     hipLaunchKernelGGL(k_rc_pack, dim3((unsigned)((n_sub + 3) / 4)), dim3(256), 0, st, rc->tokens->d_tok, rc->tokens->d_off, d_ids, rc->d_cu, b0,
-                       n_sub, rc->d_tok, d_pos, rc->d_cu_sub);
+                       n_sub, ln.d_tok, d_pos, ln.d_cu_sub);
     LM_HIP(hipGetLastError());
-    rc->forwards++;
+    rc->parts++;
     if (rc->general)
-        return lm_bert_forward_packed(&rc->gmodel, rc->d_tok, d_pos, rc->d_cu_sub, n_sub, total, max_len, rc->d_ws, rc->ws_bytes, d_out, (void*)st);
-    return lm_bert_h384_forward_packed(&rc->model, rc->d_tok, d_pos, rc->d_cu_sub, n_sub, total, max_len, rc->d_ws, rc->ws_bytes, d_out,
-                                       (void*)st);
-}
-
+        return lm_bert_forward_packed(&rc->gmodel, ln.d_tok, d_pos, ln.d_cu_sub, n_sub, total, max_len, ln.d_ws, ln.ws_bytes, d_out, (void*)st);
+    return bert_h384_forward_planned(&rc->model, ln.d_tok, d_pos, ln.d_cu_sub, n_sub, total, max_len, ln.d_ws, ln.ws_bytes, d_out, plan, (void*)st);
+}
+
+static int rc_fork(lm_recompute* rc, hipStream_t caller) {
+#if LM_RC_LANES
+    LM_HIP(hipEventRecord(rc->ev_fork, caller));
+#endif
+    return LM_OK;
+}
+
+static int rc_join(lm_recompute* rc, hipStream_t caller) {
+    int rv = LM_OK;
+#if LM_RC_LANES
+    for (int L = 1; L < RC_MAX_LANES; ++L) {
+        lm_rc_lane& ln = rc->lane[L];
+        if (!ln.busy) continue;
+        ln.busy = false;
+        hipError_t e = hipEventRecord(ln.done, ln.st);
+        if (e == hipSuccess) e = hipStreamWaitEvent(caller, ln.done, 0);
+        if (e != hipSuccess) {
+            set_error(std::string("recompute provider: joining a lane: ") + hipGetErrorString(e));
+            rv = LM_EHIP;
+        }
+    }
+#endif
+    return rv;
+}
+
+static int rc_embed_parts(lm_recompute* rc, const int32_t* d_ids, int32_t n, float* d_out, hipStream_t st);
 static int rc_embed(lm_recompute* rc, const int32_t* d_ids, int32_t n, float* d_out, hipStream_t st) {
+    const int r = rc_embed_parts(rc, d_ids, n, d_out, st);
+    if (rc->lanes == 1) return r;
+    const int j = rc_join(rc, st);
+    return r ? r : j;
+}
+
+static int rc_embed_parts(lm_recompute* rc, const int32_t* d_ids, int32_t n, float* d_out, hipStream_t st) {
     int r;
     rc->calls++;
     if (n == 0) return LM_OK;
     int64_t total;
     int32_t max_len;
+    unsigned long long split[2] = {0, 0};
     if (rc->prep_ids == d_ids && rc->prep_n == n) {
         total = rc->prep_total;
         max_len = rc->prep_maxlen;
+        split[0] = rc->prep_split[0];
+        split[1] = rc->prep_split[1];
     } else {
         if ((int64_t)n * rc->T > (int64_t)INT32_MAX) LM_FAIL(LM_EINVAL, "recompute provider: more than 2^31 tokens in one call");
         if ((r = rc_ensure_cu(rc, n, st))) return r;
         hipLaunchKernelGGL(k_rc_lengths_scan, dim3(1), dim3(1024), 0, st, rc->tokens->d_off, d_ids, n, (const unsigned long long*)nullptr,
-                           (int64_t)n, rc->T, rc->d_cu, rc->d_meta, rc->d_meta + 1);
+                           (int64_t)n, rc->T, rc->d_cu, rc->d_meta, rc->d_meta + 1, rc->lanes, rc->d_meta + 2);
         LM_HIP(hipGetLastError());
-        LM_HIP(hipMemcpyAsync(rc->h_meta, rc->d_meta, 16, hipMemcpyDeviceToHost, st));
+        LM_HIP(hipMemcpyAsync(rc->h_meta, rc->d_meta, 32, hipMemcpyDeviceToHost, st));
         LM_HIP(hipStreamSynchronize(st));
         rc->syncs++;
         total = (int64_t)rc->h_meta[0];
         max_len = (int32_t)rc->h_meta[1];
+        split[0] = rc->h_meta[2];
+        split[1] = rc->h_meta[3];
     }
     rc->prep_ids = nullptr;
     rc->prep_n = -1;
@@ -212,13 +301,28 @@
         LM_HIP(hipMemsetAsync(d_out, 0, (size_t)n * rc->hidden * 4, st));
         return LM_OK;
     }
-    if (total <= rc->max_tokens) return rc_forward(rc, d_ids, 0, n, total, max_len, d_out, st);
+    if (total <= rc->max_tokens) {
+        RcPart part[RC_MAX_LANES];
+        const int np = rc->lanes > 1 ? rc_plan_parts(n, total, rc->lanes, rc->lane_min_tokens, split, part) : 1;
+        rc->forwards++;
+        if (np == 1) return rc_forward(rc, 0, d_ids, 0, n, total, max_len, d_out, nullptr, st);
+        BertH384Plan plan;
+        if (!rc->general) plan = bert_h384_plan(&rc->model, n, total, max_len);
+        if ((r = rc_fork(rc, st))) return r;
+        for (int p = 0; p < np; ++p)
+            if ((r = rc_forward(rc, p, d_ids, part[p].b0, part[p].n, part[p].tokens, max_len, d_out + (size_t)part[p].b0 * rc->hidden,
+                                rc->general ? nullptr : &plan, st)))
+                return r;
+        return LM_OK;
+    }
     rc->h_cu.resize((size_t)n + 1);
     LM_HIP(hipMemcpyAsync(rc->h_cu.data(), rc->d_cu, ((size_t)n + 1) * 4, hipMemcpyDeviceToHost, st));
     LM_HIP(hipStreamSynchronize(st));
     rc->syncs++;
     const int32_t* cs = rc->h_cu.data();
     int32_t b0 = 0;
+    int next_lane = 0;
+    if (rc->lanes > 1 && (r = rc_fork(rc, st))) return r;
     while (b0 < n) {
         const int64_t limit = (int64_t)cs[b0] + rc->max_tokens;
         int32_t j = (int32_t)(std::upper_bound(cs + 1, cs + n + 1, limit, [](int64_t lim, int32_t v) { return lim < (int64_t)v; }) - (cs + 1));
@@ -227,7 +331,9 @@
         for (int32_t i = b0; i < j; ++i) ml = std::max(ml, cs[i + 1] - cs[i]);
         const int64_t sub_total = (int64_t)cs[j] - cs[b0];
         if (sub_total > 0) {
-            if ((r = rc_forward(rc, d_ids, b0, j - b0, sub_total, ml, d_out + (size_t)b0 * rc->hidden, st))) return r;
+            rc->forwards++;
+            if ((r = rc_forward(rc, next_lane, d_ids, b0, j - b0, sub_total, ml, d_out + (size_t)b0 * rc->hidden, nullptr, st))) return r;
+            next_lane = (next_lane + 1) % rc->lanes;
         } else {
             LM_HIP(hipMemsetAsync(d_out + (size_t)b0 * rc->hidden, 0, (size_t)(j - b0) * rc->hidden * 4, st));
         }
@@ -237,6 +343,33 @@
 }
 
 int32_t rc_width(const lm_recompute* rc) { return rc->hidden; }
+
+static int rc_set_lanes(lm_recompute* rc, int lanes) {
+#if LM_RC_LANES
+    if (lanes > 1 && !rc->ev_fork) LM_HIP(hipEventCreateWithFlags(&rc->ev_fork, hipEventDisableTiming));
+    for (int L = 1; L < RC_MAX_LANES; ++L) {
+        lm_rc_lane& ln = rc->lane[L];
+        if (L < lanes) {
+            if (!ln.st) LM_HIP(hipStreamCreateWithFlags(&ln.st, hipStreamNonBlocking));
+            if (!ln.done) LM_HIP(hipEventCreateWithFlags(&ln.done, hipEventDisableTiming));
+        } else {
+            if (ln.st) {
+                (void)hipStreamSynchronize(ln.st);
+                (void)hipStreamDestroy(ln.st);
+            }
+            if (ln.done) (void)hipEventDestroy(ln.done);
+            for (void* p : {(void*)ln.d_cu_sub, (void*)ln.d_tok, ln.d_ws})
+                if (p) (void)hipFree(p);
+            ln = lm_rc_lane{};
+        }
+    }
+    rc->lanes = lanes;
+#else
+    (void)lanes;
+    rc->lanes = 1;
+#endif
+    return LM_OK;
+}
 
 static int rc_finish_create(lm_recompute* rc, const lm_tokens* tokens, int32_t max_seq_len, int64_t max_tokens, lm_recompute** out) {
     rc->device = tokens->device;
@@ -246,10 +379,17 @@
     if (const char* ft = getenv("LEANN_MI355X_FORWARD_TOKENS"))
         if (atoll(ft) > 0) rc->max_tokens = atoll(ft);
     hipError_t e;
-    if ((e = hipMalloc((void**)&rc->d_meta, 16)) != hipSuccess || (e = hipHostMalloc((void**)&rc->h_meta, 16)) != hipSuccess) {
+    if ((e = hipMalloc((void**)&rc->d_meta, 32)) != hipSuccess || (e = hipHostMalloc((void**)&rc->h_meta, 32)) != hipSuccess) {
         set_error(std::string("lm_recompute_create: ") + hipGetErrorString(e));
         lm_recompute_free(rc);
         return LM_EHIP;
+    }
+    int lanes = LM_RC_DEFAULT_LANES;
+    if (const char* fl = getenv("LEANN_MI355X_FORWARD_LANES"))
+        if (atoi(fl) >= 1 && atoi(fl) <= RC_MAX_LANES) lanes = atoi(fl);
+    if (int r = rc_set_lanes(rc, lanes)) {
+        lm_recompute_free(rc);
+        return r;
     }
     *out = rc;
     return LM_OK;
@@ -303,7 +443,11 @@
 void lm_recompute_free(lm_recompute* rc) {
     if (!rc) return;
     (void)hipSetDevice(rc->device);
-    for (void* p : {(void*)rc->d_cu, (void*)rc->d_tok, rc->d_ws, (void*)rc->d_out, (void*)rc->d_meta})
+    (void)lm::rc_set_lanes(rc, 1);
+#if LM_RC_LANES
+    if (rc->ev_fork) (void)hipEventDestroy(rc->ev_fork);
+#endif
+    for (void* p : {(void*)rc->d_cu, (void*)rc->lane[0].d_tok, rc->lane[0].d_ws, (void*)rc->d_out, (void*)rc->d_meta})
         if (p) (void)hipFree(p);
     if (rc->h_meta) (void)hipHostFree(rc->h_meta);
     delete rc;
@@ -328,6 +472,32 @@
     return rc_embed(rc, d_ids, n, d_out, (hipStream_t)stream);
 }
 
+int lm_recompute_set_option(lm_recompute* rc, const char* name, int64_t value) {
+    using namespace lm;
+    if (!rc || !name) LM_FAIL(LM_EINVAL, "lm_recompute_set_option: NULL argument");
+    if (!strcmp(name, "lanes")) {
+        if (value < 1 || value > RC_MAX_LANES) LM_FAIL(LM_EINVAL, "lm_recompute_set_option: lanes must be 1, 2 or 3");
+        LM_HIP(hipSetDevice(rc->device));
+        return rc_set_lanes(rc, (int)value);
+    }
+    if (!strcmp(name, "lane_min_tokens")) {
+        if (value < 256 || value > INT32_MAX) LM_FAIL(LM_EINVAL, "lm_recompute_set_option: lane_min_tokens must be at least 256");
+        rc->lane_min_tokens = value;
+        return LM_OK;
+    }
+    LM_FAIL(LM_EINVAL, std::string("lm_recompute_set_option: unknown option '") + name + "'");
+}
+
+int lm_recompute_get_option(const lm_recompute* rc, const char* name, int64_t* out) {
+    using namespace lm;
+    if (!rc || !name || !out) LM_FAIL(LM_EINVAL, "lm_recompute_get_option: NULL argument");
+    if (!strcmp(name, "lanes")) *out = rc->lanes;
+    else if (!strcmp(name, "lane_min_tokens")) *out = rc->lane_min_tokens;
+    else if (!strcmp(name, "parts")) *out = rc->parts;
+    else LM_FAIL(LM_EINVAL, std::string("lm_recompute_get_option: unknown option '") + name + "'");
+    return LM_OK;
+}
+
 int lm_recompute_get_stats(const lm_recompute* rc, lm_recompute_stats* out) {
     using namespace lm;
     if (!rc || !out) LM_FAIL(LM_EINVAL, "lm_recompute_get_stats: NULL argument");
diff --git a/leann_amd/csrc/lm_search.hip b/leann_amd/csrc/lm_search.hip
--- a/leann_amd/csrc/lm_search.hip
+++ b/leann_amd/csrc/lm_search.hip
@@ -535,7 +535,7 @@
         rounds++;
         const bool native = recompute && ix->native_rc && ix->provider == lm_recompute_provider && ix->provider_user == (void*)ix->native_rc;
         if (native && (rc = rc_prepare(ix->native_rc, round_ids, ws.counters + C_NUNIQ, single ? (int64_t)ws.maxnew : ix->ws_ucap, ws.counters + C_RC_TOKENS,
-                                       ws.counters + C_RC_MAXLEN, st)) != LM_OK)
+                                       ws.counters + C_RC_MAXLEN, ws.counters + C_RC_SPLIT, st)) != LM_OK)
             return rc;
         bool do_sync = (rounds % sync_every) == 0;
         if (do_sync) {
@@ -547,7 +547,7 @@
             int32_t nu = (int32_t)hc[C_NUNIQ];
             void* d_e = nullptr;
             ix->stats.nunique += nu;
-            if (native) rc_prepared(ix->native_rc, round_ids, nu, (int64_t)hc[C_RC_TOKENS], (int32_t)hc[C_RC_MAXLEN]);
+            if (native) rc_prepared(ix->native_rc, round_ids, nu, (int64_t)hc[C_RC_TOKENS], (int32_t)hc[C_RC_MAXLEN], hc + C_RC_SPLIT);
             if (nu > 0) {
                 EvScope es(ix, &ix->ev_provider);
                 int prc = ix->provider(ix->provider_user, round_ids, nu, &d_e, (void*)st);
diff --git a/leann_amd/csrc/lm_timing.cpp b/leann_amd/csrc/lm_timing.cpp
--- a/leann_amd/csrc/lm_timing.cpp
+++ b/leann_amd/csrc/lm_timing.cpp
@@ -13,7 +13,6 @@
     hipEvent_t a, b;
     int kid, dev;
     double work;
-    void* stream;
 };
 struct Acc {
     int64_t launches = 0;
@@ -22,7 +21,6 @@
 struct DevState {
     std::vector<hipEvent_t> free_events;
     hipEvent_t last_end = nullptr;
-    void* last_stream = nullptr;
     unsigned long long* d_attn_work = nullptr;
 };
 std::atomic<unsigned> g_mask{0};
@@ -53,9 +51,12 @@
 void fold(const Pair& p) {
     DevState& ds = g_dev[p.dev];
     float ms = 0.f;
+    hipEvent_t latest = ds.last_end ? ds.last_end : p.b;
     if (hipEventElapsedTime(&ms, p.a, p.b) == hipSuccess) {
         float over = 0.f;
-        if (ds.last_end && ds.last_stream == p.stream && hipEventElapsedTime(&over, p.a, ds.last_end) == hipSuccess && over > 0.f) ms -= std::min(over, ms);
+        if (ds.last_end && hipEventElapsedTime(&over, p.a, ds.last_end) == hipSuccess && over > 0.f) ms -= std::min(over, ms);
+        float behind = 0.f;
+        if (!ds.last_end || hipEventElapsedTime(&behind, ds.last_end, p.b) != hipSuccess || behind > 0.f) latest = p.b;
         (void)hipGetLastError();
         g_acc[p.kid].launches += 1;
         g_acc[p.kid].ms += ms;
@@ -64,9 +65,9 @@
         (void)hipGetLastError();
     }
     ds.free_events.push_back(p.a);
-    if (ds.last_end) ds.free_events.push_back(ds.last_end);
-    ds.last_end = p.b;
-    ds.last_stream = p.stream;
+    if (latest != p.b) ds.free_events.push_back(p.b);
+    else if (ds.last_end) ds.free_events.push_back(ds.last_end);
+    ds.last_end = latest;
 }
 
 __global__ __launch_bounds__(256) void k_kt_attn_work(const int32_t* __restrict__ cu, int32_t n_seqs, unsigned long long hidden,
@@ -104,7 +105,7 @@
     if (!a) return;
     std::lock_guard<std::mutex> lk(g_mu);
     hipEvent_t b = get_event(dev);
-    if (b && hipEventRecord(b, (hipStream_t)st) == hipSuccess) g_pending.push_back(Pair{(hipEvent_t)a, b, kid, dev, work, st});
+    if (b && hipEventRecord(b, (hipStream_t)st) == hipSuccess) g_pending.push_back(Pair{(hipEvent_t)a, b, kid, dev, work});
     else {
         (void)hipGetLastError();
         g_dev[dev].free_events.push_back((hipEvent_t)a);
diff --git a/leann_amd/recompute.py b/leann_amd/recompute.py
--- a/leann_amd/recompute.py
+++ b/leann_amd/recompute.py
@@ -68,6 +68,22 @@
             _lib.check(_lib.load().lm_recompute_get_stats(self._native, C.byref(st)), "lm_recompute_get_stats")
         return {n: int(getattr(st, n)) for n, _ in _lib.RecomputeStats._fields_}
 
+    def set_native_option(self, name: str, value: int) -> None:
+        from . import _lib
+
+        if self.native() is None:
+            raise _lib.LeannMi355xError("this model / token store has no library-side recompute provider")
+        _lib.check(_lib.load().lm_recompute_set_option(self._native, name.encode(), int(value)), "lm_recompute_set_option")
+
+    def get_native_option(self, name: str) -> int:
+        from . import _lib
+
+        if self.native() is None:
+            raise _lib.LeannMi355xError("this model / token store has no library-side recompute provider")
+        v = C.c_int64()
+        _lib.check(_lib.load().lm_recompute_get_option(self._native, name.encode(), C.byref(v)), "lm_recompute_get_option")
+        return int(v.value)
+
     @property
     def chunks(self) -> int:
         return self._chunks + (self.native_stats()["chunks"] - self._native_chunks0 if self._native is not None else 0)
```

Measured after the change: 678.4 (median of 6 runs). 1.03x the previous value.
